# facebookresearch/brainmagick

Hardware: AMD Instinct MI355X
Metric: segments/s, 208-ch x 360-sample SimpleConv + ClipLoss training step (higher is better)
Workload: dtype f32 (fp32-accurate: operands split into 2 scaled f16 planes, 3 MFMA products, fp32 accumulate; same parity tolerances as exact fp32, see DESIGN.md §2); 1 GPU; cfg2: gwilliams2022-shaped MEG C=208 T=360, F=120 features, 27 subjects, clip_conv SimpleConv (8985590 params) + ClipLoss + Adam; batch_per_gpu=256, global_batch=256, negatives=local, parallelism=dp1, comm=none, rccl_world=1, candidate_gather=none, distinct_batches=8

## Files before the change

### brainmagick_amd/csrc/bm_common.h

```cpp
#pragma once
#include <hip/hip_runtime.h>
#include <stdint.h>
#include <stdio.h>
#include <math.h>

typedef float f32x16 __attribute__((ext_vector_type(16)));
typedef float f32x4 __attribute__((ext_vector_type(4)));

#define BM_OK 0
#define BM_ERR_ARG 1001
#define BM_ERR_WORKSPACE 1002
#define BM_ERR_UNSUPPORTED 1003

extern thread_local char bm_err_buf[512];
int bm_set_error(int code, const char* fmt, ...);
int bm_check_launch(const char* what);

#define BM_REQUIRE(cond, ...)                                   \
    do {                                                        \
        if (!(cond)) return bm_set_error(BM_ERR_ARG, __VA_ARGS__); \
    } while (0)

static inline int cdiv(long a, long b) { return (int)((a + b - 1) / b); }
static inline bool prefer_big(int n) { return (long)cdiv(n, 128) * 128 <= (long)cdiv(n, 64) * 64; }

struct BmFastDiv {
    unsigned mul, shift, d;
};
static inline BmFastDiv bm_fastdiv(unsigned d) {
    BmFastDiv f;
    f.d = d;
    unsigned l = 0;
    while ((1ull << l) < d) ++l;
    f.mul = (unsigned)((((1ull << l) - d) << 32) / d + 1);
    f.shift = l;
    return f;
}
__host__ __device__ __forceinline__ unsigned bm_div(unsigned n, const BmFastDiv& f) {
#if defined(__HIP_DEVICE_COMPILE__)
    const unsigned t = __umulhi(n, f.mul);
#else
    const unsigned t = (unsigned)(((unsigned long long)n * f.mul) >> 32);
#endif
    return f.shift == 0 ? n : (t + ((n - t) >> 1)) >> (f.shift - 1);
}
__host__ __device__ __forceinline__ int bm_floordiv(int a, int b) { return a >= 0 ? a / b : -((-a + b - 1) / b); }

#define BM_BKC 16
#define BM_WAVE 64

__device__ __forceinline__ int bm_xcd_remap(int id, int n) {
    const int q = n >> 3, r = n & 7;
    const int xcd = id & 7, slot = id >> 3;
    const int base = (xcd < r) ? xcd * (q + 1) : r * (q + 1) + (xcd - r) * q;
    return base + slot;
}

enum { BM_ACT_NONE = 0, BM_ACT_GELU = 1, BM_ACT_RELU = 2, BM_ACT_LEAKY = 3 };

__device__ __forceinline__ float bm_erff(float a) { return erff(a); }

__device__ __forceinline__ float bm_act(float z, int act, float leak) {
    if (act == BM_ACT_GELU) return 0.5f * z * (1.0f + bm_erff(z * 0.70710678118654752440f));
    if (act == BM_ACT_RELU) return !(z <= 0.f) ? z : 0.f;
    if (act == BM_ACT_LEAKY) return z > 0.f ? z : z * leak;
    return z;
}

__device__ __forceinline__ float bm_gelu_grad_fast(float z) {
    const float a = fabsf(z);
    const float t = __builtin_amdgcn_rcpf(fmaf(a, 0.24f, 1.0f));
    const float e = __builtin_amdgcn_exp2f(z * z * -0.72134752044448170368f);
    float q = -0.12508568359372038f;
    q = fmaf(q, t, 0.5545737304338939f);
    q = fmaf(q, t, -0.646070256151912f);
    q = fmaf(q, t, 0.6255898343952563f);
    q = fmaf(q, t, -0.15404857581855858f);
    q = fmaf(q, t, 0.15551350568092193f);
    q = fmaf(q, t, 0.08952744474497322f);
    const float eq = e * (q * t);
    const float base = z >= 0.f ? 1.0f - eq : eq;
    return fmaf(e, z * 0.39894228040143267794f, base);
}
#define BM_ACT_GELU_FASTGRAD 4

__device__ __forceinline__ float bm_act_grad(float z, int act, float leak) {
    if (act == BM_ACT_GELU_FASTGRAD) return bm_gelu_grad_fast(z);
    if (act == BM_ACT_GELU) {
        const float cdf = 0.5f * (1.0f + bm_erff(z * 0.70710678118654752440f));
        const float pdf = 0.39894228040143267794f * expf(-0.5f * z * z);
        return cdf + z * pdf;
    }
    if (act == BM_ACT_RELU) return !(z <= 0.f) ? 1.f : 0.f;
    if (act == BM_ACT_LEAKY) return z > 0.f ? 1.f : leak;
    return 1.f;
}

__device__ __forceinline__ float bm_wave_sum(float v) {
#pragma unroll
    for (int o = 32; o > 0; o >>= 1) v += __shfl_xor(v, o);
    return v;
}
__device__ __forceinline__ double bm_wave_sum_d(double v) {
#pragma unroll
    for (int o = 32; o > 0; o >>= 1) v += __shfl_xor(v, o);
    return v;
}
template <typename T>
__device__ __forceinline__ void bm_wave_to_lds(T v, T* sh) {
    if ((threadIdx.x & 63) == 0) sh[threadIdx.x >> 6] = v;
}
#define BM_AMAX_SHARDS 8
#define BM_AMAX_WS 16384
__device__ __forceinline__ float bm_wave_max(float v);
struct BmAmaxDst {
    float* ws;
};
__device__ __forceinline__ void bm_publish_amax_at(float m, const BmAmaxDst& dst, float* sh ,
                                                   unsigned wg ) {
    if (!dst.ws) return;
    bm_wave_to_lds(bm_wave_max(m), sh);
    __syncthreads();
    if (threadIdx.x == 0) {
        const int nw = (blockDim.x + 63) >> 6;
        float v = sh[0];
        for (int w = 1; w < nw; ++w) v = fmaxf(v, sh[w]);
        dst.ws[wg] = v;
    }
}
__device__ __forceinline__ void bm_publish_amax(float m, const BmAmaxDst& dst, float* sh) {
    bm_publish_amax_at(m, dst, sh, blockIdx.y * gridDim.x + blockIdx.x);
}
__device__ __forceinline__ void bm_publish_amax(float m, float* ws, float* sh) {
    bm_publish_amax(m, BmAmaxDst{ws}, sh);
}
__device__ __forceinline__ float bm_amax_load(const float* slot) {
    float m = slot[0];
#pragma unroll
    for (int i = 1; i < BM_AMAX_SHARDS; ++i) m = fmaxf(m, slot[i]);
    return m;
}
int bm_amax_finalize(const float* ws, int n, float* out, hipStream_t stream);
int bm_amax_finalize_rows(const float* ws, int C, int nsplit, float* out, float* rows_out, hipStream_t stream);
int bm_amax_finalize_rows_sums(const float* ws, int C, int nsplit, float* out, float* rows_out,
                               const double* sum_partial, float* sums_out, hipStream_t stream);
static inline BmAmaxDst bm_amax_dst(float* amax_out, float* amax_ws) {
    return BmAmaxDst{amax_out ? amax_ws : nullptr};
}
static inline int bm_amax_done(const BmAmaxDst& d, int nblocks, float* amax_out, hipStream_t stream) {
    return d.ws ? bm_amax_finalize(d.ws, nblocks, amax_out, stream) : BM_OK;
}

__device__ __forceinline__ float bm_wave_max(float v) {
#pragma unroll
    for (int o = 32; o > 0; o >>= 1) v = fmaxf(v, __shfl_xor(v, o));
    return v;
}
```

### brainmagick_amd/csrc/conv_h2_common.h

```cpp
#pragma once
#include <cstdlib>
#include <cstring>
#include "conv_common.h"
#include "mfma_split.h"

typedef _Float16 f16x8 __attribute__((ext_vector_type(8)));

#define HBN 192
#define HXWP 256
#define HXSLAB (2 * 2 * HXWP)
#define PACK_MAX_NK 3840

struct ConvH2Args {
    ConvNNArgs c;
    const float* x_amax;
    const float* wscale;
    BmAmaxDst y_amax;
};

template <int MW>
struct H2Simple {
    float* yb;
    const float* rb;
    int rowu, li, T;
    int row0, M;
    float bia[MW][16];
};

template <int MW, int NT, int MT, bool FULL>
__device__ __forceinline__ float h2_simple_col(const H2Simple<MW>& e, f32x16 (&acc)[MW][3], float amx) {
    if constexpr (MT < MW) {
        float rv[16];
        if (e.rb) {
#pragma unroll
            for (int r = 0; r < 16; ++r) {
                const int dr = MT * 32 + (r & 3) + 8 * (r >> 2);
                rv[r] = (FULL || e.row0 + dr < e.M) ? e.rb[(long)(e.rowu + dr) * e.T + e.li + NT * 32] : 0.f;
            }
        }
#pragma unroll
        for (int r = 0; r < 16; ++r) {
            const int dr = MT * 32 + (r & 3) + 8 * (r >> 2);
            float v = acc[MT][NT][r] + e.bia[MT][r];
            if (e.rb) v += rv[r];
            if (FULL || e.row0 + dr < e.M) {
                amx = fmaxf(amx, fabsf(v));
                e.yb[(long)(e.rowu + dr) * e.T + e.li + NT * 32] = v;
            }
        }
        return h2_simple_col<MW, NT, MT + 1, FULL>(e, acc, amx);
    }
    return amx;
}

template <int MW, bool FULL>
__device__ __forceinline__ float h2_simple_tile(const H2Simple<MW>& e, f32x16 (&acc)[MW][3], int col0, int T) {
    float amx = 0.f;
    if (col0 < T) amx = h2_simple_col<MW, 0, 0, FULL>(e, acc, amx);
    if (col0 + 32 < T) amx = h2_simple_col<MW, 1, 0, FULL>(e, acc, amx);
    if (col0 + 64 < T) amx = h2_simple_col<MW, 2, 0, FULL>(e, acc, amx);
    return amx;
}

struct H2Plain {
    float* yb;
    const float* rb;
    int rowu, li, T;
    int row0, M;
};

template <int MW, bool FULL>
__device__ __forceinline__ void h2_residual_add(const H2Plain& e, f32x16 (&acc)[MW][3], int col0, int T) {
    constexpr int NBLK = MW * 3, D = 3;
    float rv[D][16];
    const bool cok[3] = {col0 < T, col0 + 32 < T, col0 + 64 < T};
    bm_static_for<NBLK + D>([&](auto ic) __attribute__((always_inline)) {
        constexpr int i = decltype(ic)::value;
        if constexpr (i >= D) {
            constexpr int b = i - D, nt = b / MW, mt = b % MW;
            if (cok[nt]) {
#pragma unroll
                for (int r = 0; r < 16; ++r) acc[mt][nt][r] += rv[b % D][r];
            }
        }
        if constexpr (i < NBLK) {
            constexpr int nt = i / MW, mt = i % MW;
            if (cok[nt]) {
#pragma unroll
                for (int r = 0; r < 16; ++r) {
                    const int dr = mt * 32 + (r & 3) + 8 * (r >> 2);
                    rv[i % D][r] = (FULL || e.row0 + dr < e.M) ? e.rb[(long)(e.rowu + dr) * e.T + e.li + nt * 32] : 0.f;
                }
            }
        }
    });
}
template <int MW, int NT, int MT, bool FULL>
__device__ __forceinline__ float h2_plain_col(const H2Plain& e, f32x16 (&acc)[MW][3], float amx) {
    if constexpr (MT < MW) {
#pragma unroll
        for (int r = 0; r < 16; ++r) {
            const int dr = MT * 32 + (r & 3) + 8 * (r >> 2);
            const float v = acc[MT][NT][r];
            if (FULL || e.row0 + dr < e.M) {
                amx = fmaxf(amx, fabsf(v));
                e.yb[(long)(e.rowu + dr) * e.T + e.li + NT * 32] = v;
            }
        }
        return h2_plain_col<MW, NT, MT + 1, FULL>(e, acc, amx);
    }
    return amx;
}
template <int MW, bool FULL>
__device__ __forceinline__ float h2_plain_tile(const H2Plain& e, f32x16 (&acc)[MW][3], int col0, int T) {
    float amx = 0.f;
    if (col0 < T) amx = h2_plain_col<MW, 0, 0, FULL>(e, acc, amx);
    if (col0 + 32 < T) amx = h2_plain_col<MW, 1, 0, FULL>(e, acc, amx);
    if (col0 + 64 < T) amx = h2_plain_col<MW, 2, 0, FULL>(e, acc, amx);
    return amx;
}

template <int MW, int I>
__device__ __forceinline__ float h2_general_blocks(const ConvNNArgs& a, f32x16 (&acc)[MW][3], const float* ep, int b,
                                                   int m0, int rl_base, int col_base, float amx) {
    if constexpr (I < MW * 3) {
        constexpr int MT = I / 3, NT = I % 3;
        float v[16];
        float m = 0.f;
        conv_ep_store_block(a, acc[MT][NT], ep, 64 * MW, b, m0, rl_base + MT * 32, col_base + NT * 32, v, &m);
        return h2_general_blocks<MW, I + 1>(a, acc, ep, b, m0, rl_base, col_base, fmaxf(amx, m));
    }
    return amx;
}

template <int MW>
__device__ __forceinline__ void h2_tile_stats(const ConvNNArgs& a, f32x16 (&acc)[MW][3], const float* epl ,
                                              float* stats_tile , long row_stride ,
                                              int row0 , int col0, int lane) {
    const bool c0ok = col0 < a.T, c1ok = col0 + 32 < a.T, c2ok = col0 + 64 < a.T;
    const bool all_in = __builtin_amdgcn_readfirstlane(col0 - (lane & 31)) + 95 < a.T;
    const bool b4 = lane & 16, b3 = lane & 8, b2 = lane & 4, b1 = lane & 2;
    bm_static_for<MW>([&](auto mc) __attribute__((always_inline)) {
        constexpr int mt = decltype(mc)::value;
        float s1[16], s2[16];
        if (all_in) {
#pragma unroll
            for (int r = 0; r < 16; ++r) {
                const float bias = epl[mt * 32 + (r & 3) + 8 * (r >> 2)];
                const float v0 = acc[mt][0][r] + bias, v1 = acc[mt][1][r] + bias, v2 = acc[mt][2][r] + bias;
                s1[r] = (v0 + v1) + v2;
                s2[r] = fmaf(v0, v0, fmaf(v1, v1, v2 * v2));
            }
        } else {
#pragma unroll
            for (int r = 0; r < 16; ++r) {
                const float bias = epl[mt * 32 + (r & 3) + 8 * (r >> 2)];
                const float v0 = c0ok ? acc[mt][0][r] + bias : 0.f;
                const float v1 = c1ok ? acc[mt][1][r] + bias : 0.f;
                const float v2 = c2ok ? acc[mt][2][r] + bias : 0.f;
                s1[r] = (v0 + v1) + v2;
                s2[r] = fmaf(v0, v0, fmaf(v1, v1, v2 * v2));
            }
        }
#define H2_FOLD(N_, BIT_, MASK_)                                                                  \
        _Pragma("unroll") for (int i = 0; i < N_; ++i) {                                          \
            const float k1 = BIT_ ? s1[i + N_] : s1[i], g1 = BIT_ ? s1[i] : s1[i + N_];            \
            const float k2 = BIT_ ? s2[i + N_] : s2[i], g2 = BIT_ ? s2[i] : s2[i + N_];            \
            s1[i] = k1 + __shfl_xor(g1, MASK_);                                                   \
            s2[i] = k2 + __shfl_xor(g2, MASK_);                                                   \
        }
        H2_FOLD(8, b4, 16)
        H2_FOLD(4, b3, 8)
        H2_FOLD(2, b2, 4)
        H2_FOLD(1, b1, 2)
#undef H2_FOLD
        s1[0] += __shfl_xor(s1[0], 1);
        s2[0] += __shfl_xor(s2[0], 1);
        const int q = (b4 ? 8 : 0) + (b3 ? 4 : 0) + (b2 ? 2 : 0) + (b1 ? 1 : 0);
        const int row = row0 + mt * 32 + (q & 3) + 8 * (q >> 2);
        if (!(lane & 1) && row < a.M)
            *reinterpret_cast<float2*>(stats_tile + (long)row * row_stride) = float2{s1[0], s2[0]};
    });
}

template <int MW, bool RESK = false>
__device__ __forceinline__ void h2_tile_epilogue(const ConvH2Args& args, f32x16 (&acc)[MW][3], float* smem, int b, int g,
                                                 int m0, int n0, int ntile, float sx_inv, int tid, int lane, int wm,
                                                 int wn, int nl, int h, unsigned* trace_out = nullptr) {
    const ConvNNArgs& a = args.c;
    constexpr int NW = 3;
    constexpr int HBM = 64 * MW;
#ifdef HG_TRACE
    unsigned te[6];
#define H2_TE(I_) { __builtin_amdgcn_sched_barrier(0); te[I_] = (unsigned)__builtin_readcyclecounter(); __builtin_amdgcn_sched_barrier(0); }
#else
#define H2_TE(I_)
#endif
    H2_TE(0)
    float* ep = smem;
    conv_ep_stage_params(a, ep, HBM, m0, tid, 256, b);
    {
        const float* ws = args.wscale + (long)g * a.Mpad + m0;
        for (int i = tid; i < HBM; i += 256) ep[3 * HBM + i] = ws[i] * sx_inv;
    }
    __syncthreads();
    H2_TE(1)
    if constexpr (RESK) {
        const float* fl = ep + 3 * HBM + wm * (MW * 32) + 4 * h;
        const float* bl = ep + wm * (MW * 32) + 4 * h;
#pragma unroll
        for (int mt = 0; mt < MW; ++mt)
#pragma unroll
            for (int r = 0; r < 16; ++r) {
                const float f = fl[mt * 32 + (r & 3) + 8 * (r >> 2)];
                const float bb = bl[mt * 32 + (r & 3) + 8 * (r >> 2)];
#pragma unroll
                for (int nt = 0; nt < NW; ++nt) acc[mt][nt][r] = fmaf(acc[mt][nt][r], f, bb);
            }
        H2Plain e;
        e.yb = a.y_out + (long)b * a.y_bstride;
        e.rb = a.res + (long)b * a.res_bstride;
        e.rowu = m0 + wm * (MW * 32);
        e.li = 4 * h * a.T + n0 + wn * (NW * 32) + nl;
        e.T = a.T;
        e.row0 = e.rowu + 4 * h;
        e.M = a.M;
        const int col0 = n0 + wn * (NW * 32) + nl;
        float amx;
        if (m0 + HBM <= a.M) {
            h2_residual_add<MW, true>(e, acc, col0, a.T);
            amx = h2_plain_tile<MW, true>(e, acc, col0, a.T);
        } else {
            h2_residual_add<MW, false>(e, acc, col0, a.T);
            amx = h2_plain_tile<MW, false>(e, acc, col0, a.T);
        }
        bm_publish_amax(amx, args.y_amax, smem + 4 * HBM);
        return;
    }
    {
        const float* fl = ep + 3 * HBM + wm * (MW * 32) + 4 * h;
#pragma unroll
        for (int mt = 0; mt < MW; ++mt)
#pragma unroll
            for (int r = 0; r < 16; ++r) {
                const float f = fl[mt * 32 + (r & 3) + 8 * (r >> 2)];
#pragma unroll
                for (int nt = 0; nt < NW; ++nt) acc[mt][nt][r] *= f;
            }
    }
    H2_TE(2)
    if (a.stats)
        h2_tile_stats<MW>(a, acc, ep + wm * (MW * 32) + 4 * h,
                          a.stats + (long)((b * a.ntiles_n + ntile) * 2 + wn) * 2, (long)a.B * a.ntiles_n * 4,
                          m0 + wm * (MW * 32) + 4 * h, n0 + wn * (NW * 32) + nl, lane);
    const bool simple = ((a.y_pre != nullptr) != (a.y_out != nullptr)) && !a.ep_scale && a.act == BM_ACT_NONE;
    H2_TE(3)
    if (simple) {
        H2Simple<MW> e;
        e.yb = (a.y_pre ? a.y_pre : a.y_out) + (long)b * a.y_bstride;
        e.rb = (a.y_out && a.res) ? a.res + (long)b * a.res_bstride : nullptr;
        e.rowu = m0 + wm * (MW * 32);
        e.li = 4 * h * a.T + n0 + wn * (NW * 32) + nl;
        e.T = a.T;
        e.row0 = e.rowu + 4 * h;
        e.M = a.M;
        const float* epl = ep + wm * (MW * 32) + 4 * h;
#pragma unroll
        for (int mt = 0; mt < MW; ++mt)
#pragma unroll
            for (int r = 0; r < 16; ++r) e.bia[mt][r] = epl[mt * 32 + (r & 3) + 8 * (r >> 2)];
        const int col0 = n0 + wn * (NW * 32) + nl;
        const float amx = m0 + HBM <= a.M ? h2_simple_tile<MW, true>(e, acc, col0, a.T)
                                          : h2_simple_tile<MW, false>(e, acc, col0, a.T);
        H2_TE(4)
        if (a.y_out) bm_publish_amax(amx, args.y_amax, smem + 4 * HBM);
        H2_TE(5)
#ifdef HG_TRACE
        if (trace_out && blockIdx.x < 64 && lane == 0) {
            unsigned* o = trace_out + ((blockIdx.x * 4 + (threadIdx.x >> 6)) * 3) * 8;
            o[1] = te[1] - te[0]; o[2] = te[2] - te[1]; o[3] = te[3] - te[2]; o[8 + 1] = te[4] - te[3]; o[8 + 2] = te[5] - te[4];
        }
#endif
    } else {
        const float amx = h2_general_blocks<MW, 0>(a, acc, ep, b, m0, wm * (MW * 32) + 4 * h,
                                                   n0 + wn * (NW * 32) + nl, 0.f);
        bm_publish_amax(amx, args.y_amax, smem + 4 * HBM);
    }
}


#ifdef HG_TRACE
#define CH_T(I_) { __builtin_amdgcn_sched_barrier(0); tr[I_] = (unsigned)__builtin_readcyclecounter(); __builtin_amdgcn_sched_barrier(0); }
#else
#define CH_T(I_)
#endif

extern "C" int bm_conv_h2_mpad(int M);
extern "C" int bm_amax(const float* x, long n, float* out, float* ws, void* stream);
```

### brainmagick_amd/csrc/conv_nn_h2w.hip

```cpp
#include "conv_h2_common.h"

#ifdef HG_TRACE
__device__ unsigned ch_trace_buf[64 * 4 * 24];
extern "C" int bm_debug_trace_read_conv(unsigned* out) {
    return (int)hipMemcpyFromSymbol(out, HIP_SYMBOL(ch_trace_buf), sizeof(unsigned) * 64 * 4 * 24);
}
#endif

__device__ __forceinline__ void ch_split_hi(float x0, float x1, float s, unsigned& hi) {
    asm("v_fma_mixlo_f16 %0, %1, %3, 0\n\t"
        "v_fma_mixhi_f16 %0, %2, %3, 0" : "=&v"(hi) : "v"(x0), "v"(x1), "v"(s));
}
__device__ __forceinline__ void ch_split_lo(float x0, float x1, float s, unsigned hi, unsigned& lo) {
    asm("v_fma_mixlo_f16 %0, %2, %4, -%1 op_sel_hi:[0,0,1]\n\t"
        "v_fma_mixhi_f16 %0, %3, %4, -%1 op_sel:[0,0,1] op_sel_hi:[0,0,1]"
        : "=&v"(lo) : "v"(hi), "v"(x0), "v"(x1), "v"(s));
}

enum { H2R_NONE = 0, H2R_WLOAD, H2R_SPLIT, H2R_WRITE, H2R_BAR, H2R_BREAD };
struct H2RItem { int kind, arg; };
template <int KS, int J, int NB>
constexpr int h2r_nitems() {
    if (KS == 1) return 32 + 4 + 1 + NB;
    return J == 0 ? 16 + NB : J == 1 ? 16 + 4 + 1 + NB : NB;
}
template <int KS, int J, int NB>
constexpr H2RItem h2r_item(int i) {
    if (KS == 1) {
        if (i < 16) return (i & 3) < 2 ? H2RItem{H2R_SPLIT, (i >> 2) * 2 + (i & 1)} : H2RItem{H2R_WLOAD, (i >> 2) * 2 + (i & 1)};
        if (i < 18) return H2RItem{H2R_WRITE, i - 16};
        if (i < 34) { const int k = i - 18; return (k & 3) < 2 ? H2RItem{H2R_SPLIT, 8 + (k >> 2) * 2 + (k & 1)} : H2RItem{H2R_WLOAD, 8 + (k >> 2) * 2 + (k & 1)}; }
        if (i < 36) return H2RItem{H2R_WRITE, i - 34 + 2};
        if (i == 36) return H2RItem{H2R_BAR, 0};
        return H2RItem{H2R_BREAD, i - 37};
    }
    if (J == 0) return i < 16 ? H2RItem{H2R_WLOAD, i} : H2RItem{H2R_BREAD, i - 16};
    if (J == 1) {
        if (i < NB) return H2RItem{H2R_BREAD, i};
        i -= NB;
        if (i < 8) return H2RItem{H2R_SPLIT, i};
        if (i < 10) return H2RItem{H2R_WRITE, i - 8};
        if (i < 18) return H2RItem{H2R_SPLIT, i - 2};
        if (i < 20) return H2RItem{H2R_WRITE, i - 18 + 2};
        return H2RItem{H2R_BAR, 0};
    }
    return H2RItem{H2R_BREAD, i};
}

template <int KS, int MW, bool RESK = false>
__global__ __launch_bounds__(256, 1) void conv_nn_h2w_kernel(ConvH2Args args) {
    const ConvNNArgs& a = args.c;
#ifdef HG_TRACE
    const unsigned t_kernel0 = (unsigned)__builtin_readcyclecounter();
#endif
    constexpr int NW = 3;
    constexpr int HBM = 64 * MW;
    constexpr int TN = MW * NW, NS = 3 * TN;
    constexpr int NA = 2 * MW, NB = 2 * NW;
    constexpr int NF = NS - (NS + 3) / 4;
    static_assert(4 * (NA - 1) < NS, "the A loads of a stage need a slot each");
    extern __shared__ __attribute__((aligned(16))) float smem[];
    u32x4* Xs = reinterpret_cast<u32x4*>(smem);
    const int tid = threadIdx.x;
    const int lane = tid & 63;
    const int wave = __builtin_amdgcn_readfirstlane(tid >> 6);
    const int wm = wave >> 1, wn = wave & 1;
    const int nl = lane & 31;
    const int h = lane >> 5;

    int id = bm_xcd_remap(blockIdx.x, gridDim.x);
    const int mtile = id % a.ntiles_m;
    id /= a.ntiles_m;
    const int ntile = id % a.ntiles_n;
    const int b = id / a.ntiles_n;
    const int m0 = mtile * HBM;
    const int n0 = ntile * HBN;
    const int halo = (KS >> 1) * a.dil;
    const int XW = HBN + 2 * halo;

    const int g = a.widx ? a.widx[b] : 0;
    const int n16 = 2 * a.nchunk;
    float sx, sx_inv;
    bm_scale_from_amax(bm_amax_load(args.x_amax), sx, sx_inv);

    const long gslots = (long)a.nchunk * KS * 8 * a.Mpad;
    const __amdgpu_buffer_rsrc_t wr = bm_buffer_rsrc(reinterpret_cast<const u32x4*>(a.wp) + (long)g * gslots, (unsigned)(gslots * 16));
    const int wvoff = (h * a.Mpad + m0 + wm * (MW * 32) + nl) * 16;
    const int pstride = 4 * a.Mpad * 16;
    const __amdgpu_buffer_rsrc_t xr = bm_buffer_rsrc(a.x + (long)b * a.x_bstride, (unsigned)(a.Cin * a.T * 4));
    const int tcol = n0 - halo + tid;
    const int xoff0 = (tid < XW && tcol >= 0 && tcol < a.T) ? tcol * 4 : 0x40000000;
    const int crow = a.T * 4;

    f32x16 acc[MW][NW];
#pragma unroll
    for (int i = 0; i < MW; ++i)
#pragma unroll
        for (int k = 0; k < NW; ++k)
#pragma unroll
            for (int r = 0; r < 16; ++r) acc[i][k][r] = 0.f;

    float xreg[16];
    unsigned ph[8], pw[8];
    f16x8 af[2][2][MW], bf[2][2][NW];

#define H2R_LOAD_A(SET_, K_, SOFF_)                                                                       \
    af[SET_][1 - (K_) / MW][(K_) % MW] = __builtin_bit_cast(f16x8, __builtin_amdgcn_raw_buffer_load_b128(  \
        wr, wvoff + ((K_) % MW) * 512, (SOFF_) + (1 - (K_) / MW) * pstride, 0));
#define H2R_SOFF(C16_, J_) (((((C16_) >> 1) * KS + (J_)) * 8 + ((C16_) & 1) * 2) * a.Mpad * 16)
#define H2R_LOAD_X(R_, CB_) xreg[R_] = __builtin_bit_cast(float, __builtin_amdgcn_raw_buffer_load_b32(xr, (CB_) + (R_) * crow, 0, 0));
    const u32x4* xrd = Xs + h * HXWP + wn * (NW * 32) + nl;
    u32x4* xwr = Xs + tid;

    bm_static_for<16>([&](auto rc) __attribute__((always_inline)) { H2R_LOAD_X(decltype(rc)::value, xoff0) });
    bm_static_for<NA>([&](auto kc) __attribute__((always_inline)) { H2R_LOAD_A(0, decltype(kc)::value, 0) });
    bm_static_for<8>([&](auto uc) __attribute__((always_inline)) {
        constexpr int u = decltype(uc)::value;
        ch_split_hi(xreg[2 * u], xreg[2 * u + 1], sx, ph[u]);
        ch_split_lo(xreg[2 * u], xreg[2 * u + 1], sx, ph[u], pw[u]);
    });
    xwr[(0 * 2 + 0) * HXWP] = u32x4{ph[0], ph[1], ph[2], ph[3]};
    xwr[(1 * 2 + 0) * HXWP] = u32x4{pw[0], pw[1], pw[2], pw[3]};
    xwr[(0 * 2 + 1) * HXWP] = u32x4{ph[4], ph[5], ph[6], ph[7]};
    xwr[(1 * 2 + 1) * HXWP] = u32x4{pw[4], pw[5], pw[6], pw[7]};
    if (KS == 1) bm_static_for<16>([&](auto rc) __attribute__((always_inline)) { H2R_LOAD_X(decltype(rc)::value, 16 * crow + xoff0) });
    asm volatile("s_waitcnt lgkmcnt(0)\n\ts_barrier" ::: "memory");
    bm_static_for<NB>([&](auto ic) __attribute__((always_inline)) {
        constexpr int i = decltype(ic)::value;
        bf[0][i / NW][i % NW] = __builtin_bit_cast(f16x8, xrd[(i / NW) * 2 * HXWP + (i % NW) * 32]);
    });

#ifdef HG_TRACE
    unsigned tr[8], tacc[3][8];
    for (int i = 0; i < 3; ++i) for (int k = 0; k < 8; ++k) tacc[i][k] = 0;
    __builtin_amdgcn_sched_barrier(0);
    const unsigned t_loop0 = (unsigned)__builtin_readcyclecounter();
#endif
    auto stage = [&](int c16, auto jc, auto pc) __attribute__((always_inline)) {
        constexpr int j = decltype(jc)::value, par = decltype(pc)::value;
        CH_T(0)
        const bool last_chunk = c16 + 1 >= n16;
        const int nc16 = (j == KS - 1 && !last_chunk) ? c16 + 1 : c16;
        const int soff = (j == KS - 1) ? H2R_SOFF(nc16, last_chunk ? KS - 1 : 0) : H2R_SOFF(c16, j + 1);
        const u32x4* xnext = xrd + ((j == KS - 1 ? c16 + 1 : c16) & 1) * HXSLAB + (j == KS - 1 ? 0 : (j + 1) * a.dil);
        const int cb = (c16 + (KS == 1 ? 2 : 1)) * 16 * crow + xoff0;
        u32x4* xw = xwr + ((c16 + 1) & 1) * HXSLAB;
        bm_static_for<NS>([&](auto nc) __attribute__((always_inline)) {
            constexpr int n = decltype(nc)::value;
            constexpr int term = n / TN, w = n % TN, mt = w / NW, nt = w % NW;
            constexpr int pa = term == 0 ? 1 : 0, pb = term == 1 ? 1 : 0;
            acc[mt][nt] = __builtin_amdgcn_mfma_f32_32x32x16_f16(af[par][pa][mt], bf[par][pb][nt], acc[mt][nt], 0, 0, 0);
            if constexpr (n % 4 == 0) {
                if constexpr (n / 4 < NA) H2R_LOAD_A(par ^ 1, n / 4, soff)
            } else {
                constexpr int f = (n / 4) * 3 + n % 4 - 1;
                constexpr int L = h2r_nitems<KS, j, NB>();
                constexpr int i0 = (f * L + NF - 1) / NF, i1 = ((f + 1) * L + NF - 1) / NF;
                bm_static_for<i1 - i0>([&](auto ic) __attribute__((always_inline)) {
                    constexpr H2RItem it = h2r_item<KS, j, NB>(i0 + decltype(ic)::value);
                    if constexpr (it.kind == H2R_WLOAD) {
                        H2R_LOAD_X(it.arg, cb)
                    } else if constexpr (it.kind == H2R_SPLIT) {
                        constexpr int u = it.arg / 2;
                        if constexpr (it.arg % 2 == 0) ch_split_hi(xreg[2 * u], xreg[2 * u + 1], sx, ph[u]);
                        else ch_split_lo(xreg[2 * u], xreg[2 * u + 1], sx, ph[u], pw[u]);
                    } else if constexpr (it.kind == H2R_WRITE) {
                        constexpr int kg = it.arg / 2, plane = it.arg % 2;
                        if constexpr (plane == 0) xw[(0 * 2 + kg) * HXWP] = u32x4{ph[4 * kg], ph[4 * kg + 1], ph[4 * kg + 2], ph[4 * kg + 3]};
                        else xw[(1 * 2 + kg) * HXWP] = u32x4{pw[4 * kg], pw[4 * kg + 1], pw[4 * kg + 2], pw[4 * kg + 3]};
                    } else if constexpr (it.kind == H2R_BAR) {
                        asm volatile("s_waitcnt lgkmcnt(0)\n\ts_barrier" ::: "memory");
                    } else if constexpr (it.kind == H2R_BREAD) {
                        constexpr int p = it.arg / NW, q = it.arg % NW;
                        bf[par ^ 1][p][q] = __builtin_bit_cast(f16x8, xnext[p * 2 * HXWP + q * 32]);
                    }
                });
            }
            __builtin_amdgcn_sched_barrier(0);
        });
        CH_T(4)
#ifdef HG_TRACE
        tacc[j][0] += tr[4] - tr[0]; tacc[j][7] += 1;
#endif
    };
    auto chunk = [&](int c16, auto cpc) __attribute__((always_inline)) {
        constexpr int cp = decltype(cpc)::value;
        bm_static_for<KS>([&](auto jc) __attribute__((always_inline)) {
            constexpr int j = decltype(jc)::value;
            stage(c16, jc, std::integral_constant<int, (cp + j) & 1>{});
        });
    };
    for (int c16 = 0; c16 < n16; c16 += 2) {
        chunk(c16, std::integral_constant<int, 0>{});
        chunk(c16 + 1, std::integral_constant<int, KS & 1>{});
    }
#ifdef HG_TRACE
    __builtin_amdgcn_sched_barrier(0);
    const unsigned t_loop1 = (unsigned)__builtin_readcyclecounter();
    if (blockIdx.x < 64 && lane == 0)
        for (int i = 0; i < 3; ++i) for (int k = 0; k < 8; ++k) ch_trace_buf[((blockIdx.x * 4 + wave) * 3 + i) * 8 + k] = tacc[i][k];
#endif
    asm volatile("s_waitcnt vmcnt(0) lgkmcnt(0)\n\ts_barrier" ::: "memory");
#undef H2R_LOAD_A
#undef H2R_SOFF
#undef H2R_LOAD_X

#ifdef HG_TRACE
    h2_tile_epilogue<MW, RESK>(args, acc, smem, b, g, m0, n0, ntile, sx_inv, tid, lane, wm, wn, nl, h, ch_trace_buf);
#else
    h2_tile_epilogue<MW, RESK>(args, acc, smem, b, g, m0, n0, ntile, sx_inv, tid, lane, wm, wn, nl, h);
#endif
#ifdef HG_TRACE
    asm volatile("s_waitcnt vmcnt(0)" ::: "memory");
    if (blockIdx.x < 64 && lane == 0) {
        unsigned* o = ch_trace_buf + ((blockIdx.x * 4 + wave) * 3) * 8;
        o[5] = t_loop0 - t_kernel0;
        o[6] = (unsigned)__builtin_readcyclecounter() - t_loop1;
        o[8 + 5] = t_loop1 - t_loop0;
    }
#endif
}

extern "C" int bm_conv_h2_mw_for(int M) {
    int best = 5;
    long best_pad = -1;
    const int cand[3] = {5, 4, 2};
    for (int i = 0; i < 3; ++i) {
        const long bm = 64L * cand[i];
        const long pad = (long)cdiv(M, bm) * bm;
        if (best_pad < 0 || pad < best_pad) { best_pad = pad; best = cand[i]; }
    }
    return best;
}
extern "C" int bm_conv_h2_mpad(int M) {
    const int bm = 64 * bm_conv_h2_mw_for(M);
    return cdiv(M, bm) * bm;
}

extern "C" int bm_conv_h2_covers(int Cin, int M, int T, int KS, int dil) {
    if (KS != 1 && KS != 3) return 0;
    if ((KS >> 1) * dil > 16 || T <= 128) return 0;
    if ((long)Cin * T * 4 >= 0x40000000L) return 0;
    if ((long)Cin * KS > PACK_MAX_NK) return 0;
    return (long)bm_conv_h2_mpad(M) * 2 <= (long)M * 3 || M >= 96;
}

extern "C" int bm_conv_h2_stats_tiles(int B, int T) { return B * cdiv(T, HBN) * 2; }

template <int KS, int MW>
static int launch_conv_nn_h2w(ConvH2Args args, float* y_amax_out, hipStream_t stream) {
    constexpr int HBM = 64 * MW;
    const size_t lds_ep = (size_t)(4 * HBM + 4) * sizeof(float);
    const size_t lds = (size_t)(2 * HXSLAB) * 16 > lds_ep ? (size_t)(2 * HXSLAB) * 16 : lds_ep;
    const ConvNNArgs& c = args.c;
    const bool resk = KS == 3 && c.res && c.y_out && !c.y_pre && !c.ep_scale && !c.stats && c.act == BM_ACT_NONE;
    args.c.ntiles_n = cdiv(args.c.T, HBN);
    args.c.ntiles_m = args.c.Mpad / HBM;
    const long nblocks = (long)args.c.B * args.c.ntiles_n * args.c.ntiles_m;
    if (nblocks <= 0) return BM_OK;
    const bool publish = y_amax_out && args.y_amax.ws && nblocks <= BM_AMAX_WS;
    float* ws = args.y_amax.ws;
    if (!publish) args.y_amax = BmAmaxDst{nullptr};
    if (resk)
        hipLaunchKernelGGL((conv_nn_h2w_kernel<KS, MW, KS == 3>), dim3((unsigned)nblocks), dim3(256), lds, stream, args);
    else
        hipLaunchKernelGGL((conv_nn_h2w_kernel<KS, MW, false>), dim3((unsigned)nblocks), dim3(256), lds, stream, args);
    if (int rc = bm_check_launch("conv_nn_h2w")) return rc;
    if (publish) return bm_amax_done(args.y_amax, (int)nblocks, y_amax_out, stream);
    if (y_amax_out && ws)
        return bm_amax(args.c.y_out, (long)args.c.B * args.c.M * args.c.T, y_amax_out, ws, stream);
    return BM_OK;
}

extern "C" int bm_conv1d_nn_h2(const float* x, long x_bstride, const float* x_amax, const void* wpacked,
                               const int* widx, const float* bias, long bias_gstride, const float* ep_scale, const float* ep_shift,
                               const float* res, long res_bstride, float* y_pre, float* y_out, long y_bstride,
                               float* stats, int B, int Cin, int M, int T, int KS, int dil, int act, float leak,
                               int G, float* y_amax_out, float* amax_ws, void* stream) {
    BM_REQUIRE(x_amax, "conv1d_nn_h2: null x_amax");
    BM_REQUIRE(G >= 1, "conv1d_nn_h2: bad dims");
    BM_REQUIRE(!stats || (y_pre && !y_out && !ep_scale && act == BM_ACT_NONE && !res),
               "conv1d_nn_h2: per-tile statistics come with y_pre alone (the training-mode BatchNorm layers)");
    ConvH2Args args;
    ConvNNArgs& a = args.c;
    if (int e = conv_nn_fill_args(a, "conv1d_nn_h2", x, x_bstride, (const float*)wpacked, widx, bias, bias_gstride, ep_scale,
                                  ep_shift, res, res_bstride, y_pre, y_out, y_bstride, stats, B, Cin, M, T, KS, dil, act,
                                  leak))
        return e;
    BM_REQUIRE(bm_conv_h2_covers(Cin, M, T, KS, dil), "conv1d_nn_h2: shape not covered (Cin=%d M=%d T=%d KS=%d dil=%d)",
               Cin, M, T, KS, dil);
    const int mw = bm_conv_h2_mw_for(M);
    a.Mpad = bm_conv_h2_mpad(M);
    a.nchunk = cdiv(Cin, 32);
    const long f16_elems = (long)G * a.nchunk * KS * 2 * 4 * a.Mpad * 8;
    args.x_amax = x_amax;
    BM_REQUIRE(!y_amax_out || amax_ws, "conv1d_nn_h2: y_amax_out needs the amax workspace");
    if (!y_out) y_amax_out = nullptr;
    args.y_amax = bm_amax_dst(y_amax_out, amax_ws);
    args.wscale = reinterpret_cast<const float*>(reinterpret_cast<const char*>(wpacked) + f16_elems * 2);
    hipStream_t s = (hipStream_t)stream;
#define H2_DISPATCH(MW_)                                                                 \
    return KS == 1 ? launch_conv_nn_h2w<1, MW_>(args, y_amax_out, s) : launch_conv_nn_h2w<3, MW_>(args, y_amax_out, s);
    switch (mw) {
        case 5: H2_DISPATCH(5)
        case 4: H2_DISPATCH(4)
        default: H2_DISPATCH(2)
    }
#undef H2_DISPATCH
}
```

### brainmagick_amd/csrc/core.hip

```cpp
#include "bm_block.h"
#include <stdarg.h>
#include <stdlib.h>

thread_local char bm_err_buf[512] = {0};

int bm_set_error(int code, const char* fmt, ...) {
    va_list ap;
    va_start(ap, fmt);
    vsnprintf(bm_err_buf, sizeof(bm_err_buf), fmt, ap);
    va_end(ap);
    return code;
}

int bm_check_launch(const char* what) {
    hipError_t e = hipGetLastError();
    if (e != hipSuccess) return bm_set_error((int)e, "%s: launch failed: %s", what, hipGetErrorString(e));
    return BM_OK;
}

extern "C" const char* bm_last_error(void) { return bm_err_buf; }
extern "C" int bm_version(void) { return 116; }

extern "C" int bm_device_count(void) {
    int n = 0;
    hipError_t e = hipGetDeviceCount(&n);
    if (e != hipSuccess) { bm_set_error((int)e, "hipGetDeviceCount: %s", hipGetErrorString(e)); return -1; }
    return n;
}

#define FIN_THREADS 1024
#define FIN_WAVES (FIN_THREADS / 64)
__global__ __launch_bounds__(FIN_THREADS) void amax_finalize_kernel(const float* __restrict__ ws, int n,
                                                                    float* __restrict__ out) {
    __shared__ float sh[FIN_WAVES];
    bm_amax_fold<FIN_WAVES>(ws, n, out, sh);
}

int bm_amax_finalize(const float* ws, int n, float* out, hipStream_t stream) {
    if (!out) return BM_OK;
    hipLaunchKernelGGL(amax_finalize_kernel, dim3(1), dim3(FIN_THREADS), 0, stream, ws, n, out);
    return bm_check_launch("amax_finalize");
}

__global__ __launch_bounds__(FIN_THREADS) void amax_finalize_rows_kernel(const float* __restrict__ ws, int C, int nsplit,
                                                                         float* __restrict__ out,
                                                                         float* __restrict__ rows_out,
                                                                         const double* __restrict__ sum_partial,
                                                                         float* __restrict__ sums_out) {
    __shared__ float sh[FIN_WAVES];
    if (sum_partial)
        for (int c = threadIdx.x; c < C; c += FIN_THREADS) {
            double t = 0;
            for (int s = 0; s < nsplit; ++s) t += sum_partial[(long)c * nsplit + s];
            sums_out[c] = (float)t;
        }
    bm_amax_fold_rows<FIN_WAVES>(ws, C, nsplit, 1, C, out, rows_out, sh);
}

int bm_amax_finalize_rows(const float* ws, int C, int nsplit, float* out, float* rows_out, hipStream_t stream) {
    if (!out) return BM_OK;
    hipLaunchKernelGGL(amax_finalize_rows_kernel, dim3(1), dim3(FIN_THREADS), 0, stream, ws, C, nsplit, out, rows_out,
                       (const double*)nullptr, (float*)nullptr);
    return bm_check_launch("amax_finalize_rows");
}

int bm_amax_finalize_rows_sums(const float* ws, int C, int nsplit, float* out, float* rows_out,
                               const double* sum_partial, float* sums_out, hipStream_t stream) {
    hipLaunchKernelGGL(amax_finalize_rows_kernel, dim3(1), dim3(FIN_THREADS), 0, stream, ws, C, nsplit, out, rows_out,
                       sum_partial, sums_out);
    return bm_check_launch("amax_finalize_rows");
}

extern "C" int bm_amax_ws_elems(void) { return BM_AMAX_WS; }
```

### brainmagick_amd/functional.py

```python

import torch

from . import hip_ops as H



ACT_CODES = {"none": H.ACT_NONE, "gelu": H.ACT_GELU, "relu": H.ACT_RELU, "leaky": H.ACT_LEAKY}


def _c(t: torch.Tensor) -> torch.Tensor:
    return t if t.is_contiguous() else t.contiguous()


_arange_cache = {}


def _arange_i32(n: int, device, repeat: int = 1) -> torch.Tensor:
    key = (n, repeat, device.type, device.index)
    t = _arange_cache.get(key)
    if t is None:
        if len(_arange_cache) > 64:
            _arange_cache.clear()
        t = torch.arange(n, dtype=torch.int32, device=device)
        if repeat != 1:
            t = t.repeat(repeat)
        if device.type == "cuda":
            torch.cuda.current_stream(device).synchronize()
        _arange_cache[key] = t
    return t


def _conv_weight_grads(dy, x, weight, KS, dil, transposed_weight):
    dst = H.grad_destination(weight)
    B, M, T = dy.shape
    Cin = x.shape[1]
    if transposed_weight:
        out = dst if dst is not None else torch.empty(weight.shape, device=dy.device, dtype=torch.float32)
        H.gemm_nt(x, dy, B, Cin, M, T, 1, 1, out=out.view(1, Cin, M, 1))
        return out.view(weight.shape) if dst is not None else out
    if dst is not None:
        H.gemm_nt(dy, x, B, M, Cin, T, KS, dil, out=dst.view(1, M, Cin, KS))
        return dst.view(weight.shape)
    return H.gemm_nt(dy, x, B, M, Cin, T, KS, dil).view(weight.shape)


def _layer_forward(x, weight, geom, res=None, **kw):
    dil, transposed, stride, pad = geom
    if pad is not None:
        assert res is None, "the strided family has no fused residual"
        KS = weight.shape[2]
        M = weight.shape[1] if transposed else weight.shape[0]
        Tout = H.conv_out_len(x.shape[2], KS, stride, dil, pad, transposed)
        wp = H.pack_strided_rows_second(weight) if transposed else H.pack_strided_rows_first(weight)
        return H.conv_strided(x, wp, M, Tout, KS, stride, dil, pad, transposed, **kw)
    assert stride == 1
    if transposed:
        Cin, M, KS = weight.shape
        assert KS == 1, "ConvTranspose1d is only supported with kernel 1 (simpleconv.py:189)"
        wp = H.pack_weights(weight, 1, M, Cin, 1, 0, 1, M, 0, shape=(x.shape[2], dil))
    else:
        M, Cin, KS = weight.shape
        wp = H.pack_conv_fwd(weight, (x.shape[2], dil))
    if kw.get("want_stats") and getattr(wp, "_bm_mode", "") != "f16x2":
        pre, out, _ = H.conv_nn(x, wp, M, KS, dil, res=res, **dict(kw, want_stats=False))
        return pre, out, H.channel_stats(pre)
    return H.conv_nn(x, wp, M, KS, dil, res=res, **kw)


def _layer_backward(ctx, dy, x, weight, geom, res=None, publish_amax=True):
    dil, transposed, stride, pad = geom
    KS = weight.shape[2]
    Cin, T = x.shape[1], x.shape[2]
    dw = None
    if ctx.needs_input_grad[1]:
        if pad is None:
            dw = _conv_weight_grads(dy, x, weight, KS, dil, transposed)
        else:
            a, xl = (x, dy) if transposed else (dy, x)
            dw = H.conv_strided_wgrad(a, xl, KS, stride, dil, pad, out=H.grad_destination(weight)).view(weight.shape)
    dx = None
    if ctx.needs_input_grad[0]:
        if pad is not None:
            wp = H.pack_strided_rows_first(weight) if transposed else H.pack_strided_rows_second(weight)
            _, dx, _ = H.conv_strided(dy, wp, Cin, T, KS, stride, dil, pad, not transposed)
        else:
            if transposed:
                M = weight.shape[1]
                wp = H.pack_weights(weight, 1, Cin, M, 1, 0, M, 1, 0, shape=(T, dil))
            else:
                wp = H.pack_conv_dgrad(weight, (T, dil))
            _, dx, _ = H.conv_nn(dy, wp, Cin, KS, dil, res=res, publish_amax=publish_amax)
    return dx, dw


class Conv1dFn(torch.autograd.Function):

    @staticmethod
    def forward(ctx, x, weight, bias, dil: int, act: int, leak: float, transposed_weight: bool, stride: int = 1,
                pad=None):
        x, weight = _c(x), _c(weight)
        geom = (dil, transposed_weight, stride, pad)
        need_pre = act != H.ACT_NONE and any(ctx.needs_input_grad[:3])
        if need_pre and pad is None:
            pre, _, _ = _layer_forward(x, weight, geom, bias=bias, want_pre=True, want_out=False)
            out = H.affine_act_res(pre, None, None, None, act, leak)
        else:
            pre, out, _ = _layer_forward(x, weight, geom, bias=bias, act=act, leak=leak, want_pre=need_pre)
        ctx.save_for_backward(x, weight, pre)
        ctx.cfg = (geom, act, leak, bias is not None)
        return out

    @staticmethod
    def backward(ctx, dout):
        x, weight, pre = ctx.saved_tensors
        geom, act, leak, has_bias = ctx.cfg
        dout = _c(dout)
        dbias = None
        if act != H.ACT_NONE:
            dy, _, _, dbias = H.act_bn_bwd(dout, pre, None, None, None, None, False, act, leak,
                                           want_dbias=has_bias)
        else:
            dy = dout
            if has_bias:
                dbias = H.channel_sum(dy)
        dx, dw = _layer_backward(ctx, dy, x, weight, geom)
        return (dx, dw, dbias) + (None,) * 6


class ConvBNActFn(torch.autograd.Function):

    @staticmethod
    def forward(ctx, x, weight, bias, gamma, beta, running_mean, running_var, num_batches,
                training: bool, dil: int, act: int, leak: float, residual: bool, momentum: float,
                eps: float, stride: int = 1, pad=None, transposed: bool = False):
        x, weight = _c(x), _c(weight)
        geom = (dil, transposed, stride, pad)
        res = x if residual else None
        needs_grad = any(ctx.needs_input_grad[:5])
        if training:
            pre, _, stats = _layer_forward(x, weight, geom, bias=bias, want_pre=True, want_out=False, want_stats=True)
            mean, invstd, scale, shift = H.bn_finalize(stats, pre.shape[0] * pre.shape[2], gamma, beta, running_mean,
                                                       running_var, num_batches, momentum, eps)
            out = H.affine_act_res(pre, scale, shift, res, act, leak)
        else:
            mean, invstd, scale, shift = H.bn_eval_affine(gamma, beta, running_mean, running_var, eps)
            pre, out, _ = _layer_forward(x, weight, geom, res=res, bias=bias, scale=scale, shift=shift, act=act,
                                         leak=leak, want_pre=needs_grad)
        ctx.save_for_backward(x, weight, pre, scale, shift, mean, invstd)
        ctx.cfg = (geom, training, act, leak, residual, bias is not None)
        return out

    @staticmethod
    def backward(ctx, dout):
        x, weight, pre, scale, shift, mean, invstd = ctx.saved_tensors
        geom, training, act, leak, residual, has_bias = ctx.cfg
        dout = _c(dout)
        dy, dgamma, dbeta, dbias = H.act_bn_bwd(dout, pre, scale, shift, mean, invstd, training, act,
                                                leak, want_affine_grads=True, want_dbias=has_bias)
        dx, dw = _layer_backward(ctx, dy, x, weight, geom, res=dout if residual else None, publish_amax=False)
        return (dx, dw, dbias, dgamma, dbeta) + (None,) * 13


class GLUConvFn(torch.autograd.Function):

    @staticmethod
    def forward(ctx, x, weight, bias):
        x, weight = _c(x), _c(weight)
        M, Cin, KS = weight.shape
        u, _, _ = H.conv_nn(x, H.pack_conv_fwd(weight, (x.shape[2], 1)), M, KS, 1, bias=bias, want_pre=True,
                            want_out=False)
        out = H.glu_fwd(u)
        ctx.save_for_backward(x, weight, u)
        ctx.has_bias = bias is not None
        return out

    @staticmethod
    def backward(ctx, dout):
        x, weight, u = ctx.saved_tensors
        M, Cin, KS = weight.shape
        du, dbias = H.glu_bwd(_c(dout), u, want_dbias=ctx.has_bias)
        dw = _conv_weight_grads(du, x, weight, KS, 1, False) if ctx.needs_input_grad[1] else None  
        dx = None
        if ctx.needs_input_grad[0]:
            _, dx, _ = H.conv_nn(du, H.pack_conv_dgrad(weight, (du.shape[2], 1)), Cin, KS, 1, publish_amax=False)
        return dx, dw, dbias


class SubjectLayersFn(torch.autograd.Function):

    @staticmethod
    def forward(ctx, x, weights, subjects):
        x, weights = _c(x), _c(weights)
        S, C, D = weights.shape
        widx = H.index_i32(_c(subjects.to(torch.int64)), S)
        wp = H.pack_weights(weights, S, D, C, 1, C * D, 1, D, 0, shape=(x.shape[2], 1))
        _, out, _ = H.conv_nn(x, wp, D, 1, 1, widx=widx)
        ctx.save_for_backward(x, weights, subjects, widx)
        return out

    @staticmethod
    def backward(ctx, dout):
        x, weights, subjects, widx = ctx.saved_tensors
        S, C, D = weights.shape
        dout = _c(dout)
        B, _, T = x.shape
        dx = None
        if ctx.needs_input_grad[0]:
            wpt = H.pack_weights(weights, S, C, D, 1, C * D, D, 1, 0, shape=(T, 1))
            _, dx, _ = H.conv_nn(dout, wpt, C, 1, 1, widx=widx)
        dw = None
        if ctx.needs_input_grad[1]:
            order, seg = H.group_by_index(_c(subjects.to(torch.int64)), S)
            dw = torch.empty_like(weights)
            H.gemm_nt(dout, x, B, D, C, T, 1, 1, order=order, seg=seg, G=S, out=dw,
                      out_strides=(C * D, 1, D, 0))
        return dx, dw, None


class ChannelMergerFn(torch.autograd.Function):

    @staticmethod
    def forward(ctx, meg, heads, positions_u, layout_index, ban_center, ban_radius: float):
        meg, heads, positions_u = _c(meg), _c(heads), _c(positions_u)
        U, C, _ = positions_u.shape
        O, D = heads.shape[-2:]
        per_layout_heads = heads.dim() == 3
        assert not per_layout_heads or heads.shape[0] == U
        emb = H.fourier_emb(positions_u, D)
        seg = _arange_i32(U + 1, meg.device)
        scores = H.gemm_nt(heads, emb, U, O, C, D, a_strides=(O * D if per_layout_heads else 0, D),
                           x_strides=(C * D, D), seg=seg, G=U).view(U, O, C)
        weights = H.masked_softmax(scores, positions_u, ban_center, ban_radius)
        widx = H.index_i32(_c(layout_index.to(torch.int64)), U)
        wp = H.pack_weights(weights, U, O, C, 1, O * C, C, 1, 0, shape=(meg.shape[2], 1))
        _, out, _ = H.conv_nn(meg, wp, O, 1, 1, widx=widx)
        ctx.save_for_backward(meg, emb, weights, layout_index, widx)
        ctx.dims = (U, C, O, D)
        ctx.per_layout_heads = per_layout_heads
        return out

    @staticmethod
    def backward(ctx, dout):
        meg, emb, weights, layout_index, widx = ctx.saved_tensors
        U, C, O, D = ctx.dims
        dout = _c(dout)
        B, _, T = meg.shape
        dheads = None
        if ctx.needs_input_grad[1]:
            order, seg = H.group_by_index(_c(layout_index.to(torch.int64)), U)
            dweights = H.gemm_nt(dout, meg, B, O, C, T, 1, 1, order=order, seg=seg, G=U).view(U, O, C)
            dscores = H.softmax_bwd(weights, dweights)
            wp = H.pack_weights(dscores, U, O, C, 1, O * C, C, 1, 0, shape=(D, 1))
            uidx = _arange_i32(U, meg.device)
            _, per_layout, _ = H.conv_nn(emb, wp, O, 1, 1, widx=uidx)
            if ctx.per_layout_heads:
                dheads = per_layout
            else:
                dheads = H.sum_over_batch(per_layout) if U > 1 else per_layout[0]
        dmeg = None
        if ctx.needs_input_grad[0]:
            wpt = H.pack_weights(weights, U, C, O, 1, O * C, 1, C, 0, shape=(T, 1))
            _, dmeg, _ = H.conv_nn(dout, wpt, C, 1, 1, widx=widx)
        return dmeg, dheads, None, None, None, None


class FusedFrontEndFn(torch.autograd.Function):

    @staticmethod
    def forward(ctx, meg, heads, w1, b1, ws, positions_u, layout_index, subjects, ban_center, ban_radius: float):
        meg, heads, w1, ws, positions_u = _c(meg), _c(heads), _c(w1), _c(ws), _c(positions_u)
        U, C, _ = positions_u.shape
        O, Dp = heads.shape
        L = w1.shape[0]
        S, _, D = ws.shape
        B, _, T = meg.shape
        dev = meg.device
        emb = H.fourier_emb(positions_u, Dp)
        seg_u = _arange_i32(U + 1, dev)
        scores = H.gemm_nt(heads, emb, U, O, C, Dp, a_strides=(0, Dp), x_strides=(C * Dp, Dp), seg=seg_u,
                           G=U).view(U, O, C)
        wm = H.masked_softmax(scores, positions_u, ban_center, ban_radius)
        _, p, _ = H.conv_nn(wm, H.pack_conv_fwd(w1), L, 1, 1)
        bcol = (b1 if b1 is not None else torch.zeros(L, device=dev)).view(1, L, 1).expand(U, L, 1)
        xp = torch.cat([p, bcol], dim=2).repeat_interleave(S, dim=0).contiguous()
        widx_p = _arange_i32(S, dev, repeat=U)
        _, wc, _ = H.conv_nn(xp, H.pack_weights(ws, S, D, L, 1, L * D, 1, D, 0), D, 1, 1, widx=widx_p)
        bias_c = wc[:, :, C].contiguous()
        pair = H.index_i32(_c(layout_index.to(torch.int64)), U) * S + H.index_i32(_c(subjects.to(torch.int64)), S)
        wpc = H.pack_weights(wc, U * S, D, C, 1, D * (C + 1), C + 1, 1, 0, shape=(T, 1))
        _, out, _ = H.conv_nn(meg, wpc, D, 1, 1, widx=pair, bias=bias_c, bias_gstride=D)
        ctx.save_for_backward(meg, emb, wm, xp, ws, w1, pair, widx_p, wc)
        ctx.dims = (U, C, O, Dp, L, S, D)
        ctx.has_b1 = b1 is not None
        return out

    @staticmethod
    def backward(ctx, dout):
        meg, emb, wm, xp, ws, w1, pair, widx_p, wc = ctx.saved_tensors
        U, C, O, Dp, L, S, D = ctx.dims
        dout = _c(dout)
        B, _, T = meg.shape
        dev = meg.device
        P = U * S
        order, seg = H.group_by_index(pair.to(torch.int64), P)
        gaug = torch.empty(P, D, C + 1, device=dev, dtype=torch.float32)
        H.gemm_nt(dout, meg, B, D, C, T, 1, 1, order=order, seg=seg, G=P, out=gaug,
                  out_strides=(D * (C + 1), C + 1, 1, 0))
        gaug[:, :, C] = H.segment_sum_cols(H.time_sums_t(dout), order, seg).t()
        seg_p = _arange_i32(P + 1, dev)
        dws = dw1 = db1 = dheads = None
        if ctx.needs_input_grad[4]:
            t1 = H.gemm_nt(xp, gaug, P, L, D, C + 1, seg=seg_p, G=P)
            dws = (H.sum_over_batch(t1.view(U, S * L * D)) if U > 1 else t1).view(S, L, D)
        _, a, _ = H.conv_nn(gaug, H.pack_weights(ws, S, L, D, 1, L * D, D, 1, 0), L, 1, 1, widx=widx_p)
        a_u = torch.stack([H.sum_over_batch(a[u * S:(u + 1) * S]) for u in range(U)])
        if ctx.has_b1 and ctx.needs_input_grad[3]:
            db1 = H.sum_over_batch(a_u[:, :, C].contiguous()) if U > 1 else a_u[0, :, C].contiguous()
        if ctx.needs_input_grad[2]:
            dw1 = H.gemm_nt(a_u, wm, U, L, O, C, 1, 1, a_strides=(L * (C + 1), C + 1),
                            x_strides=(O * C, C)).view(L, O, 1)
        if ctx.needs_input_grad[1]:
            _, dwm, _ = H.conv_nn(a_u, H.pack_conv_dgrad(w1), O, 1, 1)
            dscores = H.softmax_bwd(wm, dwm[:, :, :C].contiguous())
            wp = H.pack_weights(dscores, U, O, C, 1, O * C, C, 1, 0, shape=(Dp, 1))
            uidx = _arange_i32(U, dev)
            _, per_layout, _ = H.conv_nn(emb, wp, O, 1, 1, widx=uidx)
            dheads = H.sum_over_batch(per_layout) if U > 1 else per_layout[0]
        dmeg = None
        if ctx.needs_input_grad[0]:
            wpt = H.pack_weights(wc, P, C, D, 1, D * (C + 1), 1, C + 1, 0, shape=(T, 1))
            _, dmeg, _ = H.conv_nn(dout, wpt, C, 1, 1, widx=pair)
        return dmeg, dheads, dw1, db1, dws, None, None, None, None, None


_CLIP_BLOCK_BYTES = 0x3f000000


def _candidate_blocks(Bc: int, K: int):
    if Bc * K * 4 < _CLIP_BLOCK_BYTES:
        return [(0, Bc)]
    rows = max(1, _CLIP_BLOCK_BYTES // (K * 4))
    if rows >= 128:
        rows -= rows % 128
    return [(r0, min(rows, Bc - r0)) for r0 in range(0, Bc, rows)]


def _clip_raw_scores(estimate, candidate, B, Bc, K):
    blocks = _candidate_blocks(Bc, K)
    if len(blocks) == 1:
        return H.gemm_nt_partials(estimate, candidate, 1, B, Bc, K, (0, K), (0, K))
    raw = torch.empty(1, B, Bc, device=estimate.device, dtype=torch.float32)
    cand2 = candidate.view(Bc, K)
    for r0, rows in blocks:
        blk = H.share_amax(candidate, cand2[r0:r0 + rows])
        H.gemm_nt(estimate, blk, 1, B, rows, K, 1, 1, a_strides=(0, K), x_strides=(0, K),
                  out=raw.view(-1)[r0:], out_strides=(0, Bc, 1, 0))
    return raw


class ClipLossFn(torch.autograd.Function):

    @staticmethod
    def forward(ctx, estimate, candidate, target_offset: int = 0, col_valid=None, symmetric: bool = False,
                normalize: bool = True):
        estimate, candidate = _c(estimate), _c(candidate)
        B, Bc = estimate.shape[0], candidate.shape[0]
        K = estimate.numel() // B
        assert candidate.numel() // Bc == K
        inv = H.clip_inv_norms(candidate) if normalize else torch.ones(Bc, device=candidate.device, dtype=torch.float32)
        ctx.normalize = normalize
        part = _clip_raw_scores(estimate, candidate, B, Bc, K)
        scores, _, dscaled, loss = H.clip_ce(part, inv, want_grad=True, want_loss=True,
                                             target_offset=target_offset, col_valid=col_valid)
        if symmetric:
            H.clip_ce_cols(scores, inv, dscaled, loss, target_offset=target_offset)
        if ctx.needs_input_grad[1]:
            ctx.save_for_backward(candidate, dscaled, estimate, scores, inv)
        else:
            ctx.save_for_backward(candidate, dscaled)
        ctx.shape = estimate.shape
        ctx.cand_shape = candidate.shape
        ctx.mark_non_differentiable(scores)
        return loss, scores

    @staticmethod
    def backward(ctx, dloss, _dscores):
        candidate, dscaled = ctx.saved_tensors[:2]
        B, Bc = dscaled.shape
        K = candidate.numel() // Bc
        alpha = _c(dloss).view(1)
        blocks = _candidate_blocks(Bc, K)
        cand2 = candidate.view(Bc, K)
        dest = None
        if ctx.needs_input_grad[0]:
            for r0, rows in blocks:
                wp = H.pack_weights(dscaled.view(-1)[r0:], 1, B, rows, 1, 0, Bc, 1, 0, alpha=alpha, shape=(K, 1))
                blk = H.share_amax(candidate, cand2[r0:r0 + rows].view(1, rows, K))
                _, dest, _ = H.conv_nn(blk, wp, B, 1, 1, res=dest, out=dest)
            dest = H.share_amax(dest, dest.view(ctx.shape))
        dcand = None
        if ctx.needs_input_grad[1]:
            estimate, scores, inv = ctx.saved_tensors[2:]
            dcand = torch.empty(Bc, K, device=candidate.device, dtype=torch.float32)
            for r0, rows in blocks:
                wpt = H.pack_weights(dscaled.view(-1)[r0:], 1, rows, B, 1, 0, 1, Bc, 0, alpha=alpha, shape=(K, 1))
                H.conv_nn(estimate.view(1, B, K), wpt, rows, 1, 1,
                          out=dcand[r0:r0 + rows] if len(blocks) > 1 else dcand)
            if ctx.normalize:
                coef = H.clip_cand_coef(dscaled, scores, inv, alpha)
                H.row_axpy_sub(dcand, cand2, coef)
            dcand = dcand.view(ctx.cand_shape)
        return dest, dcand, None, None, None, None


def clip_scores(estimate, candidate, want_probs=False):
    estimate, candidate = _c(estimate), _c(candidate)
    B, Bc = estimate.shape[0], candidate.shape[0]
    K = estimate.numel() // B
    inv = H.clip_inv_norms(candidate)
    part = _clip_raw_scores(estimate, candidate, B, Bc, K)
    scores, probs, _, _ = H.clip_ce(part, inv, want_probs=want_probs)
    return probs if want_probs else scores


def clip_forward_timed(estimate, candidate, inv, timer):
    B, Bc = estimate.shape[0], candidate.shape[0]
    K = estimate.numel() // B
    H.set_kernel_timer(timer)
    try:
        part = _clip_raw_scores(estimate, candidate, B, Bc, K)
        return H.clip_ce(part, inv, want_grad=True, want_loss=True)
    finally:
        H.set_kernel_timer(None)


class MaskedRegressionFn(torch.autograd.Function):

    @staticmethod
    def forward(ctx, estimate, output, mask, kind: str, flag=None):
        estimate, output = _c(estimate), _c(output)
        mask = None if mask is None else _c(mask)
        loss, count = H.regress_loss_fwd(estimate, output, mask, kind, flag)
        ctx.kind = kind
        ctx.save_for_backward(estimate, output, mask, count)
        ctx.mark_non_differentiable(count)
        return loss, count

    @staticmethod
    def backward(ctx, dloss, _dcount):
        estimate, output, mask, count = ctx.saved_tensors
        if not (ctx.needs_input_grad[0] or ctx.needs_input_grad[1]):
            return None, None, None, None, None
        dest, dout = H.regress_loss_bwd(estimate, output, mask, ctx.kind, _c(dloss), count,
                                        want_dout=ctx.needs_input_grad[1])
        return (dest if ctx.needs_input_grad[0] else None), dout, None, None, None


class FeatureDecodingFn(torch.autograd.Function):

    @staticmethod
    def forward(ctx, estimate, output, mask, table, weights=None, flag=None):
        estimate, output = _c(estimate), _c(output)
        mask = None if mask is None else _c(mask)
# ... 120 lines not shown
```

### brainmagick_amd/hip_ops.py

```python
import ctypes
import math
import typing as tp

import numpy as np
import torch

from ._lib import lib, check, BmHipError

ACT_NONE, ACT_GELU, ACT_RELU, ACT_LEAKY = 0, 1, 2, 3
BKC = 16

import os as _os
DEFAULT_COMPUTE_DTYPE = "f16x2"
COMPUTE_DTYPES = ("f32", "f32x3", "f16x2")
_compute_dtype = _os.environ.get("BM_COMPUTE_DTYPE", DEFAULT_COMPUTE_DTYPE)
if _compute_dtype not in COMPUTE_DTYPES:
    raise ValueError(f"BM_COMPUTE_DTYPE must be one of {COMPUTE_DTYPES}, got {_compute_dtype!r}")


def set_compute_dtype(name: str):
    global _compute_dtype
    if name not in COMPUTE_DTYPES:
        raise ValueError(f"compute dtype must be one of {COMPUTE_DTYPES}, got {name!r}")
    _compute_dtype = name


def get_compute_dtype() -> str:
    return _compute_dtype


class KernelTimer:

    def __init__(self):
        self.records: tp.List[tp.Tuple[str, float, torch.cuda.Event, torch.cuda.Event]] = []

    def launch(self, name: str, flops: float, fn):
        start = torch.cuda.Event(enable_timing=True)
        end = torch.cuda.Event(enable_timing=True)
        start.record()
        out = fn()
        end.record()
        self.records.append((name, flops, start, end))
        return out

    def summary(self) -> tp.Dict[str, tp.Dict[str, float]]:
        samples: tp.Dict[str, tp.List[float]] = {}
        flops_sum: tp.Dict[str, float] = {}
        for name, flops, start, end in self.records:
            samples.setdefault(name, []).append(start.elapsed_time(end))
            flops_sum[name] = flops_sum.get(name, 0.0) + flops
        out = {}
        for name, v in samples.items():
            med = sorted(v)[len(v) // 2]
            kept = [t for t in v if t <= 20.0 * med]
            out[name] = dict(launches=len(v), avg_ms=sum(kept) / len(kept), median_ms=med, max_ms=max(v),
                             outliers=len(v) - len(kept), flops_per_launch=flops_sum[name] / len(v))
        return out


_timer: tp.Optional[KernelTimer] = None
_MODE_SUFFIX = {"f32": "", "f32x3": "_x3", "f16x2": "_h2w"}


def set_kernel_timer(timer: tp.Optional[KernelTimer]):
    global _timer
    _timer = timer


def _timed(label, flops: float, launch):
    if _timer is None:
        return launch()
    return _timer.launch(label() if callable(label) else label, flops, launch)


def _p(t: tp.Optional[torch.Tensor]):
    return None if t is None else ctypes.c_void_p(t.data_ptr())


def _stream():
    return ctypes.c_void_p(torch.cuda.current_stream().cuda_stream)


def _req(t: torch.Tensor, name: str, dtype=torch.float32, contiguous: bool = True):
    if not isinstance(t, torch.Tensor) or not t.is_cuda:
        raise BmHipError(f"{name}: expected a GPU tensor; the brainmagick_amd hot path has no CPU "
                         "fallback (got %s)" % (t.device if isinstance(t, torch.Tensor) else type(t)))
    if t.dtype != dtype:
        raise BmHipError(f"{name}: expected dtype {dtype}, got {t.dtype}")
    if contiguous and not t.is_contiguous():
        raise BmHipError(f"{name}: expected a contiguous tensor")
    return t


def _opt(t, name, dtype=torch.float32):
    return None if t is None else _req(t, name, dtype)


_WS_KINDS = {
    "amax": ("bm_amax_ws_elems", torch.float32, False),
    "regress": ("bm_regress_workspace_bytes", torch.uint8, True),
    "encode": ("bm_meg_init_workspace_bytes", torch.uint8, True),
    "lowpass": ("bm_lowpass_workspace_bytes", torch.uint8, True),
}
_stream_workspaces: tp.Dict[tp.Any, torch.Tensor] = {}


def _stream_ws(kind: str, device) -> torch.Tensor:
    key = (kind, device, torch.cuda.current_stream(device).cuda_stream)
    ws = _stream_workspaces.get(key)
    if ws is None:
        size, dtype, zeroed = _WS_KINDS[kind]
        alloc = torch.zeros if zeroed else torch.empty
        ws = _stream_workspaces[key] = alloc(getattr(lib(), size)(), device=device, dtype=dtype)
    return ws


def conv_mpad(M: int) -> int:
    return lib().bm_conv_mpad(M)


def _note(t: torch.Tensor, attr: str, value, *checked):
    try:
        setattr(t, attr, (t._version, t.data_ptr(), value) + checked)
        t._bm_epoch = _weights_epoch
    except Exception:
        pass


def _noted(t: torch.Tensor, attr: str, need_checked: bool = False):
    note = getattr(t, attr, None)
    if note is not None and note[0] == t._version and note[1] == t.data_ptr() and (not need_checked or note[3]) and \
            (not (t.requires_grad and t.is_leaf) or getattr(t, "_bm_epoch", None) == _weights_epoch):
        return note[2]
    return None


AMAX_SHARDS = 8
amax_scans = 0


def amax(x: torch.Tensor, nonfinite_flag: tp.Optional[torch.Tensor] = None) -> torch.Tensor:
    cached = _noted(x, "_bm_amax", nonfinite_flag is not None)
    if cached is not None:
        return cached
    _req(x, "amax.x")
    global amax_scans
    amax_scans += 1
    out = torch.empty(AMAX_SHARDS, device=x.device, dtype=torch.float32)
    check(lib().bm_amax_checked(_p(x), x.numel(), _p(out), _p(_stream_ws("amax", x.device)),
                                _p(_opt(nonfinite_flag, "nonfinite_flag", torch.int32)), _stream()), "bm_amax")
    _note(x, "_bm_amax", out, nonfinite_flag is not None)
    return out


_amax_pool: tp.Dict[torch.device, tp.List[tp.Any]] = {}


def _amax_slot(t: torch.Tensor) -> tp.Optional[torch.Tensor]:
    if _compute_dtype != "f16x2" or t.numel() == 0:
        return None
    pool = _amax_pool.get(t.device)
    if pool is None or pool[1] >= pool[0].numel():
        pool = _amax_pool[t.device] = [torch.zeros(4096 * AMAX_SHARDS, device=t.device, dtype=torch.float32), 0]
    slot = pool[0][pool[1]:pool[1] + AMAX_SHARDS]
    pool[1] += AMAX_SHARDS
    _note(t, "_bm_amax", slot, False)
    return slot


def _row_amax_out(t: torch.Tensor, slot) -> tp.Optional[torch.Tensor]:
    if slot is None:
        return None
    rows = torch.empty(t.shape[1], device=t.device, dtype=torch.float32)
    _note(t, "_bm_row_amax", rows)
    return rows


def row_amax_of(t: torch.Tensor) -> tp.Optional[torch.Tensor]:
    return _noted(t, "_bm_row_amax")


def _slot_args(slot):
    return (_p(slot), _p(_stream_ws("amax", slot.device)) if slot is not None else None)


def _touched(t: torch.Tensor) -> torch.Tensor:
    for attr in ("_bm_amax", "_bm_row_amax", "_bm_inv_norms"):
        if getattr(t, attr, None) is not None:
            try:
                delattr(t, attr)
            except AttributeError:
                pass
    return t


def share_amax(src: torch.Tensor, view: torch.Tensor) -> torch.Tensor:
    if _compute_dtype != "f16x2":
        return view
    _note(view, "_bm_amax", amax(src), False)
    return view


_weights_epoch = 0
pack_launches = 0


def weights_changed():
    global _weights_epoch
    _weights_epoch += 1


class _PackPlan:
    MAX_JOBS = 512
    KEEP = 3

    def __init__(self, device):
        self.device = device
        self.entries: tp.Dict[tuple, dict] = {}
        self.table: tp.Optional[torch.Tensor] = None
        self.total_blocks = 0

    def get(self, src: torch.Tensor, geom: tuple) -> torch.Tensor:
        key = (src.data_ptr(),) + geom
        e = self.entries.get(key)
        if e is None:
            if len(self.entries) >= self.MAX_JOBS:
                self.entries.clear()
            G, M, Cin, KS = geom[:4]
            dst = torch.empty(lib().bm_packed_weight_bytes_h2(G, M, Cin, KS), device=src.device, dtype=torch.uint8)
            dst._bm_mode = "f16x2"
            dst._bm_groups = G
            e = self.entries[key] = dict(src=src, ptr=src.data_ptr(), geom=geom, dst=dst, stamp=None)
            self.table = None
        e["used"] = _weights_epoch
        if e["stamp"] != (_weights_epoch, src._version):
            self.refresh()
        return e["dst"]

    def refresh(self):
        global pack_launches
        stale = [k for k, e in self.entries.items()
                 if e["used"] < _weights_epoch - self.KEEP or e["src"].data_ptr() != e["ptr"]]
        for k in stale:
            del self.entries[k]
        if stale:
            self.table = None
        ents = list(self.entries.values())
        if not ents:
            return
        if self.table is None:
            nb = lib().bm_pack_h2_job_bytes()
            host = ctypes.create_string_buffer(nb * len(ents))
            block0 = 0
            for i, e in enumerate(ents):
                n = lib().bm_pack_h2_job_fill(ctypes.c_void_p(ctypes.addressof(host) + i * nb), _p(e["src"]),
                                              _p(e["dst"]), *e["geom"], None, block0)
                if n < 0:
                    raise BmHipError("bm_pack_h2_job_fill: bad arguments %r" % (e["geom"],))
                block0 += n
            self.table = torch.frombuffer(bytearray(host.raw), dtype=torch.uint8).to(self.device)
            self.total_blocks = block0
        max_nk = max(e["geom"][2] * e["geom"][3] for e in ents)
        check(lib().bm_pack_weights_h2_batch(_p(self.table), len(ents), self.total_blocks, max_nk, _stream()),
              "bm_pack_weights_h2_batch")
        pack_launches += 1
        for e in ents:
            e["stamp"] = (_weights_epoch, e["src"]._version)


_pack_plans: tp.Dict[tp.Tuple[str, int], _PackPlan] = {}


def _pack_plan(device) -> _PackPlan:
    key = (device.type, device.index if device.index is not None else torch.cuda.current_device())
    if key not in _pack_plans:
        _pack_plans[key] = _PackPlan(torch.device(*key))
    return _pack_plans[key]


def pack_weights(src: torch.Tensor, G: int, M: int, Cin: int, KS: int, sg: int, sm: int, sc: int,
                 sj: int, flip: bool = False, alpha: tp.Optional[torch.Tensor] = None,
                 shape: tp.Optional[tp.Tuple[int, int]] = None) -> torch.Tensor:
    _req(src, "pack_weights.src")
    mode = _compute_dtype
    if mode == "f16x2":
        if shape is not None and lib().bm_conv_h2_covers(Cin, M, shape[0], KS, shape[1]):
            if alpha is None and src.requires_grad and src.is_leaf:
                return _pack_plan(src.device).get(src, (G, M, Cin, KS, sg, sm, sc, sj, int(flip)))
            nbytes = lib().bm_packed_weight_bytes_h2(G, M, Cin, KS)
            dst = torch.empty(nbytes, device=src.device, dtype=torch.uint8)
            check(lib().bm_pack_weights_h2(_p(src), _p(dst), G, M, Cin, KS, sg, sm, sc, sj, int(flip),
                                           _p(_opt(alpha, "alpha")), _stream()), "bm_pack_weights_h2")
            global pack_launches
            pack_launches += 1
            dst._bm_mode = "f16x2"
            dst._bm_groups = G
            return dst
        mode = "f32x3"
    if mode == "f32x3":
        n = lib().bm_packed_weight_elems_x3(G, M, Cin, KS)
        dst = torch.empty(n, device=src.device, dtype=torch.bfloat16)
        check(lib().bm_pack_weights_x3(_p(src), _p(dst), G, M, Cin, KS, sg, sm, sc, sj, int(flip),
                                       _p(_opt(alpha, "alpha")), _stream()), "bm_pack_weights_x3")
        dst._bm_mode = mode
        return dst
    return pack_weights_f32(src, M, Cin, KS, sm, sc, sj, G, sg, flip, alpha)


def pack_weights_f32(src: torch.Tensor, M: int, Cin: int, KS: int, sm: int, sc: int, sj: int, G: int = 1, sg: int = 0,
                     flip: bool = False, alpha: tp.Optional[torch.Tensor] = None) -> torch.Tensor:
    _req(src, "pack_weights_f32.src")
    dst = torch.empty(lib().bm_packed_weight_elems(G, M, Cin, KS), device=src.device, dtype=torch.float32)
    check(lib().bm_pack_weights(_p(src), _p(dst), G, M, Cin, KS, sg, sm, sc, sj, int(flip), _p(_opt(alpha, "alpha")),
                                _stream()), "bm_pack_weights")
    return dst


def pack_conv_fwd(weight: torch.Tensor, shape=None) -> torch.Tensor:
    M, Cin, KS = weight.shape
    return pack_weights(weight, 1, M, Cin, KS, 0, Cin * KS, KS, 1, shape=shape)


def pack_conv_dgrad(weight: torch.Tensor, shape=None) -> torch.Tensor:
    M, Cin, KS = weight.shape
    return pack_weights(weight, 1, Cin, M, KS, 0, KS, Cin * KS, 1, flip=True, shape=shape)


def _conv_outputs(x: torch.Tensor, M: int, T: int, want_pre: bool, want_out: bool, stats_shape=None):
    def new(shape, want=True):
        return torch.empty(shape, device=x.device, dtype=torch.float32) if want and shape is not None else None
    return new((x.shape[0], M, T), want_pre), new((x.shape[0], M, T), want_out), new(stats_shape)


def conv_nn(x: torch.Tensor, wpacked: torch.Tensor, M: int, KS: int = 1, dil: int = 1,
            widx: tp.Optional[torch.Tensor] = None, bias=None, scale=None, shift=None, res=None,
            act: int = ACT_NONE, leak: float = 0., want_pre: bool = False, want_out: bool = True,
            want_stats: bool = False, out: tp.Optional[torch.Tensor] = None, bias_gstride: int = 0,
            publish_amax: bool = True):
    _req(x, "conv_nn.x")
    mode = getattr(wpacked, "_bm_mode", "f32")
    _req(wpacked, "conv_nn.w", {"f32": torch.float32, "f16x2": torch.uint8}.get(mode, torch.bfloat16))
    B, Cin, T = x.shape
    channel_major = want_stats and mode == "f16x2"
    stats_shape = None if not want_stats else (M, lib().bm_conv_h2_stats_tiles(B, T), 2) if channel_major else \
        (lib().bm_conv_stats_tiles(B, T), M, 2)
    y_pre, y_out, stats = _conv_outputs(x, M, T, want_pre, want_out and out is None, stats_shape)
    if channel_major:
        stats._bm_channel_major = True
    if out is not None:
        _req(out, "conv_nn.out")
        assert want_out and out.numel() == B * M * T, (out.shape, (B, M, T))
        y_out = _touched(out)
    if res is not None:
        _req(res, "conv_nn.res")
        assert res.shape == (B, M, T), (res.shape, (B, M, T))
    common = (_p(_opt(widx, "widx", torch.int32)), _p(_opt(bias, "bias")), bias_gstride, _p(_opt(scale, "scale")),
              _p(_opt(shift, "shift")), _p(res), M * T, _p(y_pre), _p(y_out), M * T, _p(stats), B, Cin, M, T,
              KS, dil, act, leak)
    if mode == "f16x2":
        x_amax = amax(x)
        y_slot = _amax_slot(y_out) if (y_out is not None and publish_amax) else None

        def launch():
            check(lib().bm_conv1d_nn_h2(_p(x), Cin * T, _p(x_amax), _p(wpacked), *common, wpacked._bm_groups,
                                        *_slot_args(y_slot), _stream()), "bm_conv1d_nn_h2")
    else:
        fn = {"f32": lib().bm_conv1d_nn, "f32x3": lib().bm_conv1d_nn_x3}[mode]

        def launch():
            check(fn(_p(x), Cin * T, _p(wpacked), *common, _stream()), f"bm_conv1d_nn[{mode}]")

    def label():
        if mode == "f16x2":
            tile = f"{KS},{lib().bm_conv_h2_mw_for(M)}"
        else:
            tile = (lib().bm_conv_mt_for if mode == "f32" else lib().bm_conv_x3_mt_for)(M)
        return f"conv_nn{_MODE_SUFFIX[mode]}_kernel<{tile}>"
    _timed(label, 2.0 * B * T * M * Cin * KS, launch)
    return y_pre, y_out, stats


def conv_out_len(T: int, KS: int, stride: int, dil: int, pad: int, transposed: bool) -> int:
    Tout = lib().bm_conv1d_out_len(T, KS, stride, dil, pad, int(transposed))
    if Tout < 1:
        if transposed:
            raise RuntimeError(f"ConvTranspose1d: input of {T} samples (kernel {KS}, stride {stride}, dilation {dil}, "
                               f"padding {pad}) gives an output of {Tout} samples. Output size is too small")
        raise RuntimeError(f"Calculated padded input size per channel: ({T + 2 * pad}). Kernel size: "
                           f"({dil * (KS - 1) + 1}). Kernel size can't be greater than actual input size")
    return Tout


def pack_strided_rows_first(weight: torch.Tensor) -> torch.Tensor:
    R, C, KS = weight.shape
    return pack_weights_f32(weight, R, C, KS, C * KS, KS, 1)


def pack_strided_rows_second(weight: torch.Tensor) -> torch.Tensor:
    C, R, KS = weight.shape
    return pack_weights_f32(weight, R, C, KS, KS, R * KS, 1)


def conv_strided(x: torch.Tensor, wpacked: torch.Tensor, M: int, Tout: int, KS: int, stride: int, dil: int, pad: int,
                 transposed: bool, bias=None, scale=None, shift=None, act: int = ACT_NONE, leak: float = 0.,
                 want_pre: bool = False, want_out: bool = True, want_stats: bool = False):
    _req(x, "conv_strided.x")
    _req(wpacked, "conv_strided.w")
    B, Cin, T = x.shape
    if Tout < 1:
        raise RuntimeError(f"conv_strided: output length {Tout} < 1")
    y_pre, y_out, stats = _conv_outputs(
        x, M, Tout, want_pre, want_out,
        (lib().bm_conv_strided_stats_tiles(B, Tout, stride, int(transposed)), M, 2) if want_stats else None)
    fn = lib().bm_conv1d_transposed if transposed else lib().bm_conv1d_strided
    name = "conv_transposed_kernel" if transposed else "conv_strided_kernel"

    def launch():
        check(fn(_p(x), Cin * T, _p(wpacked), _p(_opt(bias, "bias")), _p(_opt(scale, "scale")), _p(_opt(shift, "shift")),
                 _p(y_pre), _p(y_out), M * Tout, _p(stats), B, Cin, M, T, Tout, KS, stride, dil, pad, act, leak,
                 _stream()), "bm_conv1d_transposed" if transposed else "bm_conv1d_strided")
    taps = KS if not transposed else -(-KS // stride)
    _timed(f"{name}<K={KS},s={stride}>", 2.0 * B * (Tout if not transposed else T * stride) * M * Cin * taps, launch)
    return y_pre, y_out, stats


def conv_strided_wgrad(a: torch.Tensor, xl: torch.Tensor, KS: int, stride: int, dil: int, pad: int,
                       out: tp.Optional[torch.Tensor] = None, nsplit: tp.Optional[int] = None) -> torch.Tensor:
    _req(a, "conv_strided_wgrad.a")
    _req(xl, "conv_strided_wgrad.xl")
    S, R, U = a.shape
    S2, Q, L = xl.shape
    assert S == S2, (a.shape, xl.shape)
    if out is None:
        out = torch.empty(R, Q, KS, device=a.device, dtype=torch.float32)
    else:
        _req(out, "conv_strided_wgrad.out")
        assert out.numel() == R * Q * KS
        _touched(out)
    if nsplit is None:
        nsplit = lib().bm_conv1d_strided_wgrad_suggest_splits(R, Q, KS, S, U)
    part = out if nsplit == 1 else torch.empty(nsplit * R * Q * KS, device=a.device, dtype=torch.float32)

    def launch():
        check(lib().bm_conv1d_strided_wgrad(_p(a), R * U, _p(xl), Q * L, _p(part), S, R, Q, U, L, KS, stride, dil, pad,
                                            nsplit, _stream()), "bm_conv1d_strided_wgrad")
    _timed(f"conv_strided_wgrad_kernel<K={KS},s={stride}>", 2.0 * S * U * R * Q * KS, launch)
    if part is not out:
        check(lib().bm_reduce_splits(_p(part), _p(out), 1, nsplit, R, Q, KS, R * Q * KS, Q * KS, KS, 1, _stream()),
              "bm_reduce_splits")
    return out


_index_err: tp.Dict[torch.device, torch.Tensor] = {}
_CHECK_INDICES_NOW = _os.environ.get("BM_CHECK_INDICES", "0") == "1"


def index_error_flag(device) -> torch.Tensor:
    device = torch.device(device)
    if device.index is None:
        device = torch.device("cuda", torch.cuda.current_device())
    flag = _index_err.get(device)
    if flag is None:
        flag = torch.zeros(3, device=device, dtype=torch.int32)
        _index_err[device] = flag
    return flag


def raise_if_index_error(device=None):
    flags = list(_index_err.values()) if device is None else [index_error_flag(device)]
    for flag in flags:
        if int(flag[0].item()) != 0:
            flag[0:1].zero_()
            raise IndexError("subject / layout index out of range for the weight table "
                             "(bm/models/common.py:57 would raise in `weights.gather`)")


def index_i32(idx: torch.Tensor, G: int) -> torch.Tensor:
    _req(idx, "index_i32.idx", torch.int64)
    out = torch.empty(idx.numel(), device=idx.device, dtype=torch.int32)
    check(lib().bm_index_to_i32(_p(idx), idx.numel(), G, _p(out), _p(index_error_flag(idx.device)),
                                _stream()), "bm_index_to_i32")
    if _CHECK_INDICES_NOW:
        raise_if_index_error(idx.device)
    return out


def group_by_index(idx: torch.Tensor, G: int):
    _req(idx, "group_by_index.idx", torch.int64)
    B = idx.numel()
    order = torch.empty(B, device=idx.device, dtype=torch.int32)
    seg = torch.empty(G + 1, device=idx.device, dtype=torch.int32)
    check(lib().bm_group_by_index(_p(idx), B, G, _p(order), _p(seg), _p(index_error_flag(idx.device)),
                                  _stream()), "bm_group_by_index")
    return order, seg


_NT_SUFFIX = {"f32": "", "f32x3": "_x3"}


def _nt_plan(M, Cn, KS, S, T, G, dil, grouped, a_strides, x_strides, nsplit=None, partials=False):
    L = lib()
    family, swapped = _compute_dtype, False
    if family == "f16x2":
        family = "f32x3"
        if partials:
            if L.bm_gemm_nt_h2_covers(M, Cn, 1, S, T, 1, 1, 0):
                dense = S == 1 and tuple(a_strides) == (0, T) and tuple(x_strides) == (0, T)
                family = "scores" if dense and L.bm_clip_scores_h2_covers(M, Cn, T) else "h2"
        elif a_strides[1] == T and x_strides[1] == T and \
                (S == 1 or (a_strides[0] == M * T and x_strides[0] == Cn * T)):
            covered = bool(L.bm_gemm_nt_h2_covers(M, Cn, KS, S, T, G, dil, int(grouped)))
            swapped = not covered and KS == 1 and bool(L.bm_gemm_nt_h2_covers(Cn, M, KS, S, T, G, dil, int(grouped)))
            if swapped:
                M, Cn = Cn, M
            if covered or swapped:
                family = "h2_grouped" if grouped else "h2_rows"
    if nsplit is None:
        if family == "scores":
            nsplit = L.bm_clip_scores_h2_suggest_splits(M, Cn, T)
        elif partials:
            nsplit = L.bm_gemm_nt_h2_suggest_splits(M, Cn, 1, S, T) if family == "h2" else \
                L.bm_clip_suggest_splits(M, Cn, S, T)
        elif family in _NT_SUFFIX:
            nsplit = L.bm_gemm_nt_suggest_splits(M, Cn, KS, S, T, G)
        else:
            nsplit = L.bm_gemm_nt_h2_suggest_splits_grouped(M, Cn, KS, S, T, G)
    return family, swapped, nsplit


def _nt_launch(family, label, a, x, part, S, G, M, Cn, T, KS, dil, a_strides, x_strides, order, seg, nsplit):
    L = lib()
    if family in _NT_SUFFIX:
        fn = L.bm_gemm_nt if family == "f32" else L.bm_gemm_nt_x3

        def launch():
            check(fn(_p(a), a_strides[0], a_strides[1], _p(x), x_strides[0], x_strides[1],
                     _p(_opt(order, "order", torch.int32)), _p(_opt(seg, "seg", torch.int32)), _p(part), S,
                     G, M, Cn, T, KS, dil, nsplit, _stream()), "bm_gemm_nt")
    else:
        a_amax, x_amax = amax(a), amax(x)
        a_rows = row_amax_of(a) if family == "h2_rows" else None
        if a_rows is not None and a_rows.numel() != M:
            a_rows = None

        def launch():
            if family == "scores":
                check(L.bm_clip_scores_h2(_p(a), _p(a_amax), _p(x), _p(x_amax), _p(part), M, Cn, T, nsplit, _stream()),
                      "bm_clip_scores_h2")
            elif family == "h2_grouped":
                check(L.bm_gemm_nt_h2_grouped(_p(a), a_strides[0], a_strides[1], _p(a_amax), _p(x), x_strides[0],
                                              x_strides[1], _p(x_amax), _p(_opt(order, "order", torch.int32)),
                                              _p(_opt(seg, "seg", torch.int32)), _p(part), S, G, M, Cn, T, nsplit,
                                              _stream()), "bm_gemm_nt_h2_grouped")
            elif family == "h2_rows":
                check(L.bm_gemm_nt_h2_rows(_p(a), a_strides[0], a_strides[1], _p(a_amax), _p(a_rows), _p(x),
                                           x_strides[0], x_strides[1], _p(x_amax), _p(part), S, M, Cn, T, KS, dil,
                                           nsplit, _stream()), "bm_gemm_nt_h2")
            else:
                check(L.bm_gemm_nt_h2(_p(a), a_strides[0], a_strides[1], _p(a_amax), _p(x), x_strides[0],
                                      x_strides[1], _p(x_amax), _p(part), S, M, Cn, T, KS, dil, nsplit, _stream()),
                      "bm_gemm_nt_h2")
    _timed(label.format(_NT_SUFFIX.get(family, "_h2w")), 2.0 * S * T * M * Cn * KS, launch)


def gemm_nt(a: torch.Tensor, x: torch.Tensor, S: int, M: int, Cn: int, T: int, KS: int = 1,
            dil: int = 1, a_strides=None, x_strides=None, order=None, seg=None, G: int = 1,
            out: tp.Optional[torch.Tensor] = None, out_strides=None, nsplit: tp.Optional[int] = None):
    _req(a, "gemm_nt.a")
    _req(x, "gemm_nt.x")
    if a_strides is None:
        a_strides = (M * T, T)
    if x_strides is None:
        x_strides = (Cn * T, T)
    if out_strides is None:
        out_strides = (M * Cn * KS, Cn * KS, KS, 1)
    if out is None:
        out = torch.empty(G, M, Cn, KS, device=a.device, dtype=torch.float32)
    else:
        _touched(out)
    grouped = order is not None or seg is not None
    family, swapped, nsplit = _nt_plan(M, Cn, KS, S, T, G, dil, grouped, a_strides, x_strides, nsplit)
    if swapped:
        a, x, M, Cn, a_strides, x_strides = x, a, Cn, M, x_strides, a_strides
        out_strides = (out_strides[0], out_strides[2], out_strides[1], out_strides[3])
    canonical = tuple(out_strides) == (M * Cn * KS, Cn * KS, KS, 1)
    if nsplit == 1 and canonical:
        part = out
    else:
        part = torch.empty(G * nsplit * M * Cn * KS, device=a.device, dtype=torch.float32)
    _nt_launch(family, f"gemm_nt{{}}_kernel<KS={KS}>", a, x, part, S, G, M, Cn, T, KS, dil, a_strides, x_strides,
               order, seg, nsplit)
    if part is not out:
        check(lib().bm_reduce_splits(_p(part), _p(out), G, nsplit, M, Cn, KS, *out_strides,
                                     _stream()), "bm_reduce_splits")
    return out


class _DirectArmed:
    depth = 0

    @property
    def on(self):
        return self.depth > 0


_direct_armed = _DirectArmed()


class direct_grads_armed:

    def __enter__(self):
        _direct_armed.depth += 1
        return self

    def __exit__(self, *exc):
        _direct_armed.depth -= 1
        return False


def grad_destination(param: torch.Tensor) -> tp.Optional[torch.Tensor]:
    dst = getattr(param, "_bm_grad_dst", None)
    if dst is None or dst[1][0] or param.grad is not None or not _direct_armed.on:
        return None
    dst[1][0] = True
    return dst[0]


def gemm_nt_partials(a, x, S, M, Cn, T, a_strides, x_strides, nsplit=None):
    _req(a, "gemm_nt.a")
    _req(x, "gemm_nt.x")
    family, _, nsplit = _nt_plan(M, Cn, 1, S, T, 1, 1, False, a_strides, x_strides, nsplit, partials=True)
    part = torch.empty(nsplit, M, Cn, device=a.device, dtype=torch.float32)
    _nt_launch(family, "clip_scores:gemm_nt{}", a, x, part, S, 1, M, Cn, T, 1, 1, a_strides, x_strides, None, None, nsplit)
    return part


def sum_over_batch(x: torch.Tensor) -> torch.Tensor:
    _req(x, "sum_over_batch.x")
    B = x.shape[0]
    out = torch.empty(x.shape[1:], device=x.device, dtype=torch.float32)
    check(lib().bm_sum_over_batch(_p(x), _p(out), B, out.numel(), _stream()), "bm_sum_over_batch")
    return out


def bn_finalize(stats, count: int, gamma, beta, running_mean, running_var, num_batches,
                momentum: float, eps: float):
    _req(stats, "bn_finalize.stats")
    channel_major = getattr(stats, "_bm_channel_major", False)
    (C, ntiles, _) = stats.shape if channel_major else (stats.shape[1], stats.shape[0], 2)
    mean, invstd, scale, shift = (torch.empty(C, device=stats.device, dtype=torch.float32)
                                  for _ in range(4))
    check((lib().bm_bn_finalize_cm if channel_major else lib().bm_bn_finalize)(_p(stats), ntiles, C, count, _p(_opt(gamma, "gamma")),
                               _p(_opt(beta, "beta")), _p(_opt(running_mean, "running_mean")),
                               _p(_opt(running_var, "running_var")),
                               _p(_opt(num_batches, "num_batches", torch.int64)), momentum, eps,
                               _p(mean), _p(invstd), _p(scale), _p(shift), _stream()),
          "bm_bn_finalize")
    return mean, invstd, scale, shift


def bn_eval_affine(gamma, beta, running_mean, running_var, eps: float):
    _req(running_mean, "running_mean")
    C = running_mean.numel()
    mean, invstd, scale, shift = (torch.empty(C, device=running_mean.device, dtype=torch.float32)
                                  for _ in range(4))
    check(lib().bm_bn_eval_affine(C, _p(_opt(gamma, "gamma")), _p(_opt(beta, "beta")),
                                  _p(running_mean), _p(_req(running_var, "running_var")), eps,
                                  _p(mean), _p(invstd), _p(scale), _p(shift), _stream()),
          "bm_bn_eval_affine")
    return mean, invstd, scale, shift


def affine_act_res(y, scale, shift, res, act: int, leak: float = 0.):
    _req(y, "affine_act_res.y")
    B, C, T = y.shape
    out = torch.empty_like(y)
    check(lib().bm_affine_act_res(_p(y), _p(_opt(scale, "scale")), _p(_opt(shift, "shift")),
                                  _p(_opt(res, "res")), _p(out), B, C, T, act, leak, *_slot_args(_amax_slot(out)),
                                  _stream()), "bm_affine_act_res")
    return out


# ... 1162 lines not shown
```

### brainmagick_amd/models/common.py

```python
from functools import partial
import math
import typing as tp

import torch
from torch import nn

from .. import functional as BF
from .. import hip_ops as H


class ScaledEmbedding(nn.Module):
    def __init__(self, num_embeddings: int, embedding_dim: int, scale: float = 10.):
        super().__init__()
        self.embedding = nn.Embedding(num_embeddings, embedding_dim)
        self.embedding.weight.data /= scale
        self.scale = scale

    @property
    def weight(self):
        return self.embedding.weight * self.scale

    def forward(self, x):
        return self.embedding(x) * self.scale


class SubjectLayers(nn.Module):
    def __init__(self, in_channels: int, out_channels: int, n_subjects: int, init_id: bool = False):
        super().__init__()
        self.weights = nn.Parameter(torch.randn(n_subjects, in_channels, out_channels))
        if init_id:
            assert in_channels == out_channels
            self.weights.data[:] = torch.eye(in_channels)[None]
        self.weights.data *= 1 / in_channels**0.5

    def forward(self, x, subjects):
        return BF.SubjectLayersFn.apply(x, self.weights, subjects)

    def __repr__(self):
        S, C, D = self.weights.shape
        return f"SubjectLayers({C}, {D}, {S})"


class _Activation(nn.Module):
    def __init__(self, kind: str, leak: float = 0.):
        super().__init__()
        self.kind = kind
        self.leak = leak

    @property
    def code(self) -> int:
        return BF.ACT_CODES[self.kind]

    def extra_repr(self):
        return self.kind + (f", {self.leak}" if self.kind == "leaky" else "")


def make_activation(gelu: bool, relu_leakiness: float) -> tp.Callable[[], _Activation]:
    if gelu:
        return partial(_Activation, "gelu")
    if relu_leakiness:
        return partial(_Activation, "leaky", relu_leakiness)
    return partial(_Activation, "relu")


class _GLU(nn.Module):
    """Marker for nn.GLU(dim=1) (fused in GLUConvFn)."""


class LayerScale(nn.Module):
    def __init__(self, channels: int, init: float = 0.1, boost: float = 5.):
        super().__init__()
        self.scale = nn.Parameter(torch.zeros(channels, requires_grad=True))
        self.scale.data[:] = init / boost
        self.boost = boost

    def forward(self, x):
        return (self.boost * self.scale[:, None]) * x


class ConvSequence(nn.Module):

    def __init__(self, channels: tp.Sequence[int], kernel: int = 4, dilation_growth: int = 1,
                 dilation_period: tp.Optional[int] = None, stride: int = 2,
                 dropout: float = 0.0, leakiness: float = 0.0, groups: int = 1,
                 decode: bool = False, batch_norm: bool = False, dropout_input: float = 0,
                 skip: bool = False, scale: tp.Optional[float] = None, rewrite: bool = False,
                 activation_on_last: bool = True, post_skip: bool = False, glu: int = 0,
                 glu_context: int = 0, glu_glu: bool = True, activation: tp.Any = None) -> None:
        super().__init__()
        dilation = 1
        channels = tuple(channels)
        self.skip = skip
        self.sequence = nn.ModuleList()
        self.glus = nn.ModuleList()
        if activation is None:
            activation = partial(_Activation, "leaky", leakiness)
        self._plan: tp.List[dict] = []
        Conv = nn.Conv1d if not decode else nn.ConvTranspose1d
        strided = stride != 1 or kernel % 2 != 1 or decode
        for k, (chin, chout) in enumerate(zip(channels[:-1], channels[1:])):
            layers: tp.List[nn.Module] = []
            is_last = k == len(channels) - 2
            plan = dict(dilation=1, act=None, bn=None, glu=None, pre=None, post=[])
            if dilation_growth > 1:
                assert kernel % 2 != 0, "Supports only odd kernel with dilation for now"
            if k == 0 and dropout_input:
                assert 0 < dropout_input < 1
                layers.append(nn.Dropout(dropout_input))
                plan["pre"] = layers[-1]
            if dilation_period and (k % dilation_period) == 0:
                dilation = 1
            pad = kernel // 2 * dilation
            layers.append(Conv(chin, chout, kernel, stride, pad, dilation=dilation, groups=groups if k > 0 else 1))
            plan["conv"] = layers[-1]
            plan["dilation"] = dilation
            plan["strided"] = (stride, pad, decode) if strided else None
            dilation *= dilation_growth
            if activation_on_last or not is_last:
                if batch_norm:
                    layers.append(nn.BatchNorm1d(num_features=chout))
                    plan["bn"] = layers[-1]
                act = activation()
                layers.append(act)
                plan["act"] = act
                if dropout:
                    layers.append(nn.Dropout(dropout))
                    plan["post"].append(("dropout", layers[-1]))
                if rewrite:
                    layers += [nn.Conv1d(chout, chout, 1), _Activation("leaky", leakiness)]
                    plan["post"].append(("rewrite", layers[-2], layers[-1]))
            if chin == chout and skip:
                if scale is not None:
                    layers.append(LayerScale(chout, scale))
                    plan["post"].append(("scale", layers[-1]))
                if post_skip:
                    layers.append(Conv(chout, chout, 1, groups=chout, bias=False))
                    plan["post"].append(("post_skip", layers[-1]))
            self.sequence.append(nn.Sequential(*layers))
            if glu and (k + 1) % glu == 0:
                ch = 2 * chout if glu_glu else chout
                act = _GLU() if glu_glu else activation()
                self.glus.append(
                    nn.Sequential(
                        nn.Conv1d(chout, ch, 1 + 2 * glu_context, padding=glu_context), act))
                plan["glu"] = act
            else:
                self.glus.append(None)
            self._plan.append(plan)

    def _conv_layer(self, x, plan, code, leak, fused_residual):
        conv, bn = plan["conv"], plan["bn"]
        stride, pad, decode = plan["strided"] or (1, None, False)
        G = conv.groups
        cin, cout = conv.in_channels // G, conv.out_channels // G
        outs = []
        count0 = bn.num_batches_tracked.clone() if bn is not None and G > 1 else None
        for g in range(G):
            if G == 1:
                xg, w, b, sl = x, conv.weight, conv.bias, None
            else:
                xg = x[:, g * cin:(g + 1) * cin].contiguous()
                w = conv.weight[g * cin:(g + 1) * cin] if decode else conv.weight[g * cout:(g + 1) * cout]
                b = conv.bias[g * cout:(g + 1) * cout] if conv.bias is not None else None
                sl = slice(g * cout, (g + 1) * cout)
            if bn is not None:
                bnp = (bn.weight, bn.bias, bn.running_mean, bn.running_var) if sl is None else \
                    (bn.weight[sl], bn.bias[sl], bn.running_mean[sl], bn.running_var[sl])
                count = bn.num_batches_tracked if g == G - 1 else count0.clone()
                outs.append(BF.ConvBNActFn.apply(
                    xg, w, b, *bnp, count, self.training, plan["dilation"], code, leak, fused_residual, bn.momentum,
                    bn.eps, stride, pad, decode))
            else:
                outs.append(BF.Conv1dFn.apply(xg, w, b, plan["dilation"], code, leak, decode, stride, pad))
        return outs[0] if G == 1 else torch.cat(outs, dim=1)

    def forward(self, x: tp.Any) -> tp.Any:
        for module_idx, module in enumerate(self.sequence):
            plan = self._plan[module_idx]
            conv = plan["conv"]
            act = plan["act"]
            code = act.code if act is not None else H.ACT_NONE
            leak = act.leak if act is not None else 0.
            residual = self.skip and conv.in_channels == conv.out_channels
            old_x = x
            if plan["pre"] is not None:
                x = plan["pre"](x)
            fused_residual = residual and not plan["post"] and plan["pre"] is None and plan["strided"] is None
            x = self._conv_layer(x, plan, code, leak, fused_residual)
            for op in plan["post"]:
                if op[0] == "dropout":
                    x = op[1](x)
                elif op[0] == "rewrite":
                    x = BF.Conv1dFn.apply(x, op[1].weight, op[1].bias, 1, op[2].code, op[2].leak, False)
                elif op[0] == "scale":
                    x = op[1](x)
                else:
                    x = x * op[1].weight.view(1, -1, 1)
            if plan["strided"] is not None:
                residual = self.skip and x.shape == old_x.shape
            if residual and not (fused_residual and plan["bn"] is not None):
                x = _AddFn.apply(x if x.is_contiguous() else x.contiguous(), old_x)
            glu = self.glus[module_idx]
            if glu is not None:
                gconv = glu[0]
                if isinstance(glu[1], _GLU):
                    x = BF.GLUConvFn.apply(x, gconv.weight, gconv.bias)
                else:
                    x = BF.Conv1dFn.apply(x, gconv.weight, gconv.bias, 1, glu[1].code, glu[1].leak,
                                          False)
        return x


class _AddFn(torch.autograd.Function):
    @staticmethod
    def forward(ctx, y, res):
        return H.affine_act_res(y.contiguous(), None, None, res.contiguous(), H.ACT_NONE)

    @staticmethod
    def backward(ctx, dout):
        return dout, dout


class PositionGetter:
    INVALID = -0.1

    def __init__(self) -> None:
        self._cache: tp.Dict[int, torch.Tensor] = {}
        self._invalid_names: tp.Set[str] = set()
        self._device_cache: tp.Dict[tp.Any, tp.Tuple[torch.Tensor, torch.Tensor]] = {}
        self._layout_set_cache: tp.Dict[tp.Any, torch.Tensor] = {}
        self._layout_ids: tp.Dict[int, int] = {}
        self._layout_bytes: tp.Dict[bytes, int] = {}

    def get_recording_layout(self, recording) -> torch.Tensor:
        index = recording.recording_index
        if index in self._cache:
            return self._cache[index]
        if getattr(recording, "layout", None) is not None:
            positions = torch.as_tensor(recording.layout, dtype=torch.float32)
        else:
            positions = self._layout_from_mne(recording.mne_info)
        self._cache[index] = positions
        return positions

    def _layout_from_mne(self, info) -> torch.Tensor:
        import mne
        layout = mne.find_layout(info)
        slot_of = {name: k for k, name in enumerate(layout.names)}
        found = [(ch, slot_of[name.rsplit("-", 1)[0]]) for ch, name in enumerate(info.ch_names)
                 if name.rsplit("-", 1)[0] in slot_of]
        self._invalid_names.update(name.rsplit("-", 1)[0] for name in info.ch_names
                                   if name.rsplit("-", 1)[0] not in slot_of)
        positions = torch.full((len(info.ch_names), 2), self.INVALID)
        if found:
            channels, slots = zip(*found)
            xy = torch.as_tensor(layout.pos[list(slots), :2], dtype=torch.float64)
            lo, hi = xy.min(0).values, xy.max(0).values
            positions[list(channels)] = ((xy - lo) / (hi - lo)).float()
        return positions

    def get_positions(self, batch):
        meg = batch.meg
        B, C, T = meg.shape
        positions = torch.full((B, C, 2), self.INVALID, device=meg.device)
        for idx in range(len(batch)):
            rec_pos = self.get_recording_layout(batch._recordings[idx])
            positions[idx, :len(rec_pos)] = rec_pos.to(meg.device)
        return positions

    def get_unique_layouts(self, batch, n_channels: int, device):
        rec_ids = tuple(batch._recordings[i].recording_index for i in range(len(batch)))
        key = (rec_ids, n_channels, str(device))
        hit = self._device_cache.get(key)
        if hit is not None:
            return hit
        slots: tp.Dict[int, int] = {}
        first: tp.List[int] = []
        index: tp.List[int] = []
        for idx, rec_id in enumerate(rec_ids):
            rec_key = self._layout_ids.get(rec_id)
            if rec_key is None:
                raw = self.get_recording_layout(batch._recordings[idx]).contiguous().numpy().tobytes()
                rec_key = self._layout_ids[rec_id] = self._layout_bytes.setdefault(raw, len(self._layout_bytes))
            slot = slots.get(rec_key)
            if slot is None:
                slot = slots[rec_key] = len(first)
                first.append(idx)
            index.append(slot)
        set_key = (tuple(slots), n_channels, str(device))
        positions_u = self._layout_set_cache.get(set_key)
        if positions_u is None:
            rows = []
            for idx in first:
                pos = torch.full((n_channels, 2), self.INVALID)
                rec_pos = self.get_recording_layout(batch._recordings[idx])
                pos[:len(rec_pos)] = rec_pos
                rows.append(pos)
            positions_u = torch.stack(rows).to(device)
            if len(self._layout_set_cache) >= 64:
                self._layout_set_cache.pop(next(iter(self._layout_set_cache)))
            self._layout_set_cache[set_key] = positions_u
        layout_index = torch.tensor(index, dtype=torch.int64)
        if torch.device(device).type == "cuda":
            layout_index = layout_index.pin_memory().to(device, non_blocking=True)
        else:
            layout_index = layout_index.to(device)
        if len(self._device_cache) >= 64:
            self._device_cache.pop(next(iter(self._device_cache)))
        self._device_cache[key] = (positions_u, layout_index)
        return positions_u, layout_index

    def is_invalid(self, positions):
        return (positions == self.INVALID).all(dim=-1)


class FourierEmb(nn.Module):
    def __init__(self, dimension: int = 256, margin: float = 0.2):
        super().__init__()
        n_freqs = (dimension // 2)**0.5
        assert int(n_freqs ** 2 * 2) == dimension
        self.dimension = dimension
        self.margin = margin

    def forward(self, positions):
        return H.fourier_emb(positions.contiguous(), self.dimension, self.margin)


class ChannelDropout(nn.Module):

    N_TESTS = 100

    def __init__(self, dropout: float = 0.1, rescale: bool = True):
        super().__init__()
        self.dropout = dropout
        self.rescale = rescale
        self.position_getter = PositionGetter()
        self.ban_center_override: tp.Optional[torch.Tensor] = None

    def _centers(self, n: int, device) -> torch.Tensor:
        if self.ban_center_override is not None:
            return self.ban_center_override.to(device, torch.float32).view(1, 2).expand(n, 2)
        return torch.rand(n, 2, device=device)

    def forward(self, meg, batch):
        if not self.dropout:
            return meg
        B, C, T = meg.shape
        positions_u, layout_index = self.position_getter.get_unique_layouts(batch, C, meg.device)
        valid_u = (~self.position_getter.is_invalid(positions_u)).float()
        factor_u = valid_u
        if self.training:
            kept = ((positions_u - self._centers(1, meg.device)[0]).norm(dim=-1) > self.dropout).float()
            factor_u = factor_u * kept
            if self.rescale:
                centers = self._centers(self.N_TESTS, meg.device)
                dist = (positions_u[None] - centers[:, None, None, :]).norm(dim=-1)
                proba_kept = torch.zeros_like(valid_u)
                for n in range(self.N_TESTS):
                    proba_kept += (dist[n] > self.dropout).float() / self.N_TESTS
                factor_u = factor_u / (1e-8 + proba_kept)
        return meg * factor_u[layout_index][:, :, None]


class ChannelMerger(nn.Module):
    def __init__(self, chout: int, pos_dim: int = 256,
                 dropout: float = 0, usage_penalty: float = 0.,
                 n_subjects: int = 200, per_subject: bool = False):
        super().__init__()
        assert pos_dim % 4 == 0
        self.position_getter = PositionGetter()
        self.per_subject = per_subject
        if self.per_subject:
            self.heads = nn.Parameter(torch.randn(n_subjects, chout, pos_dim, requires_grad=True))
        else:
            self.heads = nn.Parameter(torch.randn(chout, pos_dim, requires_grad=True))
        self.heads.data /= pos_dim ** 0.5
        self.dropout = dropout
        self.embedding = FourierEmb(pos_dim)
        self.usage_penalty = usage_penalty
        self._penalty = torch.tensor(0.)
        self.ban_center_override: tp.Optional[torch.Tensor] = None

    @property
    def training_penalty(self):
        return self._penalty.to(next(self.parameters()).device)

    def layouts_and_ban(self, meg, batch):
        B, C, T = meg.shape
        positions_u, layout_index = self.position_getter.get_unique_layouts(batch, C, meg.device)
        ban_center, radius = None, 0.
        if self.training and self.usage_penalty > 0.:
            self._penalty = torch.tensor(float(self.usage_penalty))
        if self.training and self.dropout:
            if self.ban_center_override is not None:
                ban_center = self.ban_center_override.to(meg.device, torch.float32)
            else:
                ban_center = torch.rand(2, device=meg.device)
            radius = float(self.dropout)
        return positions_u, layout_index, ban_center, radius

    def forward(self, meg, batch):
        positions_u, layout_index, ban_center, radius = self.layouts_and_ban(meg, batch)
        if self.per_subject:
            n_subjects = self.heads.shape[0]
            subjects = BF.H.index_i32(batch.subject_index.to(meg.device, torch.int64).contiguous(),
                                      n_subjects).to(torch.int64)
            pairs, inverse = torch.unique(layout_index * n_subjects + subjects, return_inverse=True)
            return BF.ChannelMergerFn.apply(meg, self.heads[pairs % n_subjects].contiguous(),
                                            positions_u[pairs // n_subjects].contiguous(), inverse.contiguous(),
                                            ban_center, radius)
        return BF.ChannelMergerFn.apply(meg, self.heads, positions_u, layout_index, ban_center,
                                        radius)


def pad_multiple(x: torch.Tensor, base: int):
    length = x.shape[-1]
    target = math.ceil(length / base) * base
    return torch.nn.functional.pad(x, (0, target - length))


class DualPathRNN(nn.Module):

    def __init__(self, channels: int, depth: int, inner_length: int = 10):
        super().__init__()
        self.lstms = nn.ModuleList([nn.LSTM(channels, channels, 1) for _ in range(depth * 4)])
        self.inner_length = inner_length

    def forward(self, x: torch.Tensor) -> torch.Tensor:
        length = x.shape[-1]
        seq = pad_multiple(x, self.inner_length).permute(2, 0, 1).contiguous()
        steps, batch, channels = seq.shape
        chunks = steps // self.inner_length
        vendor_rnn = torch.backends.cudnn.enabled
        torch.backends.cudnn.enabled = False
        try:
            for k, lstm in enumerate(self.lstms):
                out = lstm(seq)[0]
                if k % 2 == 0:
                    out = out.view(self.inner_length, chunks, batch, channels).transpose(0, 1) \
                        .reshape(steps, batch, channels)
                seq = seq + out
                if k % 2 == 1:
                    seq = seq.flip(0)
        finally:
            torch.backends.cudnn.enabled = vendor_rnn
        return seq[:length].permute(1, 2, 0).contiguous()
```

### brainmagick_amd/models/simpleconv.py

```python
import random
import typing as tp

import torch
from torch import nn

from .common import (
    ConvSequence, ScaledEmbedding, SubjectLayers, ChannelMerger, ChannelDropout, DualPathRNN, make_activation)
from .. import functional as BF
from .. import hip_ops as H


_FUSE_FRONT_END = True


class SimpleConv(nn.Module):

    def __init__(self, in_channels: tp.Dict[str, int], out_channels: int, hidden: tp.Dict[str, int],
                 depth: int = 4, concatenate: bool = False, linear_out: bool = False,
                 complex_out: bool = False, kernel_size: int = 5, growth: float = 1.,
                 dilation_growth: int = 2, dilation_period: tp.Optional[int] = None, skip: bool = False,
                 post_skip: bool = False, scale: tp.Optional[float] = None, rewrite: bool = False,
                 groups: int = 1, glu: int = 0, glu_context: int = 0, glu_glu: bool = True,
                 gelu: bool = False, dual_path: int = 0, conv_dropout: float = 0.0,
                 dropout_input: float = 0.0, batch_norm: bool = False, relu_leakiness: float = 0.0,
                 n_subjects: int = 200, subject_dim: int = 64, subject_layers: bool = False,
                 subject_layers_dim: str = "input", subject_layers_id: bool = False,
                 embedding_scale: float = 1.0, n_fft: tp.Optional[int] = None, fft_complex: bool = True,
                 merger: bool = False, merger_pos_dim: int = 256, merger_channels: int = 270,
                 merger_dropout: float = 0.2, merger_penalty: float = 0., merger_per_subject: bool = False,
                 dropout: float = 0., dropout_rescale: bool = True, initial_linear: int = 0,
                 initial_depth: int = 1, initial_nonlin: bool = False, subsample_meg_channels: int = 0):
        super().__init__()
        if set(in_channels) != set(hidden):
            raise ValueError("Channels and hidden keys must match "
                             f"({set(in_channels.keys())} and {set(hidden.keys())})")
        if n_fft is not None:
            raise NotImplementedError(
                "SimpleConv option n_fft (torchaudio STFT front end) is outside the MI355X hot path: no grid of the "
                "paper uses it (SURVEY.md §2.2), and torchaudio being absent from this image the reference itself "
                "cannot run it here, so there would be nothing to hold an implementation to")
        if "meg" not in in_channels:
            raise ValueError("SimpleConv needs a 'meg' input (the sensor front end is built around it)")
        if kernel_size % 2 != 1:
            raise AssertionError("For padding to work, this must be verified")
        if linear_out and complex_out:
            raise AssertionError("linear_out and complex_out are exclusive")
        self.out_channels = out_channels
        self._concatenate = concatenate
        activation = make_activation(gelu, relu_leakiness)
        in_channels, hidden = dict(in_channels), dict(hidden)

        width = in_channels["meg"]
        self.dropout = ChannelDropout(dropout, dropout_rescale) if dropout > 0. else None
        self.subsampled_meg_channels: tp.Optional[list] = None
        if subsample_meg_channels:
            self._subsample(width, subsample_meg_channels)
        width = self._build_front_end(
            width, activation, hidden["meg"], n_subjects,
            merger=dict(on=merger, channels=merger_channels, pos_dim=merger_pos_dim, dropout=merger_dropout,
                        penalty=merger_penalty, per_subject=merger_per_subject),
            linear=dict(width=initial_linear, depth=initial_depth, nonlin=initial_nonlin),
            subject=dict(layers=subject_layers, where=subject_layers_dim, init_id=subject_layers_id,
                         emb_dim=subject_dim, emb_scale=embedding_scale))

        in_channels["meg"] = width
        if concatenate:
            in_channels = {"concat": sum(in_channels.values())}
            hidden = {"concat": sum(hidden.values())}
        widths = {name: [in_channels[name]] + [int(round(hidden[name] * growth ** k)) for k in range(depth)]
                  for name in in_channels}
        stack_kw = dict(kernel=kernel_size, stride=1, leakiness=relu_leakiness, dropout=conv_dropout,
                        dropout_input=dropout_input, batch_norm=batch_norm, dilation_growth=dilation_growth,
                        groups=groups, dilation_period=dilation_period, skip=skip, post_skip=post_skip,
                        scale=scale, rewrite=rewrite, glu=glu, glu_context=glu_context, glu_glu=glu_glu,
                        activation=activation)
        top = sum(w[-1] for w in widths.values())
        self.dual_path = DualPathRNN(top, dual_path) if dual_path else None
        if linear_out:
            self.final = nn.ConvTranspose1d(top, out_channels, 1, 1, 0)
        elif complex_out:
            self.final = nn.Sequential(nn.Conv1d(top, 2 * top, 1), activation(),
                                       nn.ConvTranspose1d(2 * top, out_channels, 1, 1, 0))
        else:
            assert len(widths) == 1, "if no linear_out, there must be a single branch."
            self.final = None
            stack_kw["activation_on_last"] = False
            next(iter(widths.values()))[-1] = out_channels
        self.encoders = nn.ModuleDict({name: ConvSequence(w, **stack_kw) for name, w in widths.items()})

    def _subsample(self, n_sensors: int, keep_n: int):
        order = list(range(n_sensors))
        random.Random(1234).shuffle(order)
        self.subsampled_meg_channels = order[:keep_n]
        keep = torch.zeros(1, n_sensors, 1)
        keep[:, self.subsampled_meg_channels] = 1.
        self.register_buffer("_channel_keep", keep, persistent=False)

    def _build_front_end(self, width: int, activation, hidden: int, n_subjects: int, merger: dict,
                         linear: dict, subject: dict) -> int:
        self.merger = self.initial_linear = self.subject_layers = self.subject_embedding = None
        if merger["on"]:
            self.merger = ChannelMerger(merger["channels"], pos_dim=merger["pos_dim"], dropout=merger["dropout"],
                                        usage_penalty=merger["penalty"], n_subjects=n_subjects,
                                        per_subject=merger["per_subject"])
            width = merger["channels"]
        if linear["width"]:
            layers: tp.List[nn.Module] = [nn.Conv1d(width, linear["width"], 1)]
            for _ in range(linear["depth"] - 1):
                layers += [activation(), nn.Conv1d(linear["width"], linear["width"], 1)]
            if linear["nonlin"]:
                layers.append(activation())
            self.initial_linear = nn.Sequential(*layers)
            width = linear["width"]
        if subject["layers"]:
            out = {"hidden": hidden, "input": width}[subject["where"]]
            self.subject_layers = SubjectLayers(width, out, n_subjects, subject["init_id"])
            width = out
        if subject["emb_dim"]:
            self.subject_embedding = ScaledEmbedding(n_subjects, subject["emb_dim"], subject["emb_scale"])
            width += subject["emb_dim"]
        return width

    def _front_end_is_linear_chain(self) -> bool:
        return (self.merger is not None and self.subject_layers is not None and self.initial_linear is not None
                and len(self.initial_linear) == 1 and self.subsampled_meg_channels is None
                and not self.merger.per_subject)

    def forward(self, inputs, batch):
        subjects = batch.subject_index
        length = next(iter(inputs.values())).shape[-1]
        x = inputs["meg"]
        if not x.is_cuda:
            raise RuntimeError("brainmagick_amd.SimpleConv runs on the MI355X HIP path only; got a "
                               f"{x.device} tensor (there is no CPU fallback)")
        if x.dtype != torch.float32:
            raise TypeError(f"SimpleConv expects fp32 inputs like the reference, got {x.dtype}")

        if self.subsampled_meg_channels is not None:
            x = x * self._channel_keep
        if self.dropout is not None:
            x = self.dropout(x, batch)
        fused = self._front_end_is_linear_chain() and _FUSE_FRONT_END
        if fused:
            positions_u, layout_index, ban_center, radius = self.merger.layouts_and_ban(x, batch)
            fused = positions_u.shape[0] * self.subject_layers.weights.shape[0] <= x.shape[0]
        self.front_end_fused = fused
        if fused:
            conv = self.initial_linear[0]
            x = BF.FusedFrontEndFn.apply(x, self.merger.heads, conv.weight, conv.bias, self.subject_layers.weights,
                                         positions_u, layout_index, subjects, ban_center, radius)
        elif self.merger is not None and self._front_end_is_linear_chain() and _FUSE_FRONT_END:
            x = BF.ChannelMergerFn.apply(x, self.merger.heads, positions_u, layout_index, ban_center, radius)
        elif self.merger is not None:
            x = self.merger(x, batch)
        if fused:
            pass
        elif self.initial_linear is not None:
            mods = list(self.initial_linear)
            i = 0
            while i < len(mods):
                conv = mods[i]
                act = mods[i + 1] if i + 1 < len(mods) and not isinstance(mods[i + 1], nn.Conv1d) \
                    else None
                x = BF.Conv1dFn.apply(x, conv.weight, conv.bias, 1,
                                      act.code if act is not None else H.ACT_NONE,
                                      act.leak if act is not None else 0., False)
                i += 2 if act is not None else 1
        if self.subject_layers is not None and not fused:
            x = self.subject_layers(x, subjects)
        if self.subject_embedding is not None:
            emb = self.subject_embedding(subjects)[:, :, None]
            x = torch.cat([x, emb.expand(-1, -1, length)], dim=1)
        inputs["meg"] = x

        if self._concatenate:
            x = self.encoders["concat"](torch.cat([v for _, v in sorted(inputs.items())], dim=1))
        elif len(self.encoders) == 1:
            x = self.encoders["meg"](x)
        else:
            x = torch.cat([self.encoders[name](v) for name, v in sorted(inputs.items())], dim=1)
        if self.dual_path is not None:
            x = self.dual_path(x)
        if self.final is not None:
            if isinstance(self.final, nn.ConvTranspose1d):
                x = BF.Conv1dFn.apply(x, self.final.weight, self.final.bias, 1, H.ACT_NONE, 0., True)
            else:
                conv, act, tconv = self.final[0], self.final[1], self.final[2]
                x = BF.Conv1dFn.apply(x, conv.weight, conv.bias, 1, act.code, act.leak, False)
                x = BF.Conv1dFn.apply(x, tconv.weight, tconv.bias, 1, H.ACT_NONE, 0., True)
        assert x.shape[-1] >= length
        return x if x.shape[-1] == length else x[:, :, :length]
```

### include/bm_hip.h

```cpp
#ifndef BM_HIP_H
#define BM_HIP_H
#ifdef __cplusplus
extern "C" {
#endif

#define BM_ACT_NONE 0
#define BM_ACT_GELU 1
#define BM_ACT_RELU 2
#define BM_ACT_LEAKY 3

int bm_version(void);
const char* bm_last_error(void);
int bm_device_count(void);

int bm_conv_mt_for(int M);
int bm_conv_mpad(int M);
int bm_conv_stats_tiles(int B, int T);
long bm_packed_weight_elems(int G, int M, int Cin, int KS);
int bm_pack_weights(const float* src, float* dst, int G, int M, int Cin, int KS, long sg, long sm,
                    long sc, long sj, int flip, const float* alpha_ptr, void* stream);
int bm_group_by_index(const long* idx, int B, int G, int* order, int* seg, int* err_flag, void* stream);
int bm_index_to_i32(const long* idx, int B, int G, int* out, int* err_flag, void* stream);
int bm_reduce_splits(const float* part, float* out, int G, int nsplit, int M, int Cn, int KS, long sg,
                     long sm, long sc, long sj, void* stream);
int bm_sum_over_batch(const float* x, float* out, int B, long n, void* stream);

int bm_conv1d_nn(const float* x, long x_bstride, const float* wpacked, const int* widx,
                 const float* bias, long bias_gstride, const float* ep_scale, const float* ep_shift, const float* res,
                 long res_bstride, float* y_pre, float* y_out, long y_bstride, float* stats, int B,
                 int Cin, int M, int T, int KS, int dil, int act, float leak, void* stream);

int bm_conv1d_out_len(int T, int KS, int stride, int dil, int pad, int transposed);
int bm_conv_strided_stats_tiles(int B, int Tout, int stride, int transposed);
int bm_conv1d_strided(const float* x, long x_bstride, const float* wpacked, const float* bias,
                      const float* ep_scale, const float* ep_shift, float* y_pre, float* y_out, long y_bstride,
                      float* stats, int B, int Cin, int M, int T, int Tout, int KS, int stride, int dil, int pad,
                      int act, float leak, void* stream);
int bm_conv1d_transposed(const float* x, long x_bstride, const float* wpacked, const float* bias,
                         const float* ep_scale, const float* ep_shift, float* y_pre, float* y_out, long y_bstride,
                         float* stats, int B, int Cin, int M, int T, int Tout, int KS, int stride, int dil, int pad,
                         int act, float leak, void* stream);
int bm_conv1d_strided_wgrad_suggest_splits(int R, int Q, int KS, int S, int U);
int bm_conv1d_strided_wgrad(const float* a, long a_sstride, const float* xl, long xl_sstride, float* part, int S,
                            int R, int Q, int U, int L, int KS, int stride, int dil, int pad, int nsplit,
                            void* stream);

int bm_lstm_layer_fwd(const float* whh0, const float* whh1, const float* gx0, const float* gx1, float* y,
                      float* gates0, float* gates1, float* c0, float* c1, int H, int B, int T, int dirs,
                      void* stream);
int bm_lstm_layer_bwd(const float* whh0, const float* whh1, const float* dy, const float* gates0,
                      const float* gates1, const float* c0, const float* c1, float* dg0, float* dg1,
                      float* dc0, float* dc1, int H, int B, int T, int dirs, void* stream);

long bm_packed_weight_elems_x3(int G, int M, int Cin, int KS);
int bm_pack_weights_x3(const float* src, void* dst, int G, int M, int Cin, int KS, long sg, long sm,
                       long sc, long sj, int flip, const float* alpha_ptr, void* stream);
int bm_conv1d_nn_x3(const float* x, long x_bstride, const void* wpacked, const int* widx,
                    const float* bias, long bias_gstride, const float* ep_scale, const float* ep_shift, const float* res,
                    long res_bstride, float* y_pre, float* y_out, long y_bstride, float* stats, int B,
                    int Cin, int M, int T, int KS, int dil, int act, float leak, void* stream);
int bm_gemm_nt_x3(const float* a, long a_sstride, long a_rstride, const float* x, long x_sstride,
                  long x_rstride, const int* order, const int* seg, float* part, int S, int G, int M,
                  int Cn, int T, int KS, int dil, int nsplit, void* stream);
int bm_conv_x3_mt_for(int M);
int bm_conv_x3_mpad(int M);

int bm_conv_h2_mw_for(int M);
int bm_conv_h2_mpad(int M);
int bm_conv_h2_covers(int Cin, int M, int T, int KS, int dil);
long bm_packed_weight_bytes_h2(int G, int M, int Cin, int KS);
int bm_pack_weights_h2(const float* src, void* dst, int G, int M, int Cin, int KS, long sg, long sm, long sc,
                       long sj, int flip, const float* alpha_ptr, void* stream);
int bm_pack_h2_job_bytes(void);
int bm_pack_h2_job_fill(void* job, const float* src, void* dst, int G, int M, int Cin, int KS, long sg, long sm,
                        long sc, long sj, int flip, const float* alpha_ptr, int block0);
int bm_pack_weights_h2_batch(const void* jobs_dev, int njobs, int total_blocks, int max_nk, void* stream);
int bm_amax_ws_elems(void);
int bm_amax(const float* x, long n, float* out, float* amax_ws, void* stream);
int bm_amax_checked(const float* x, long n, float* out, float* amax_ws, int* nonfinite_flag, void* stream);
int bm_conv_h2_stats_tiles(int B, int T);
int bm_conv1d_nn_h2(const float* x, long x_bstride, const float* x_amax, const void* wpacked, const int* widx,
                    const float* bias, long bias_gstride, const float* ep_scale, const float* ep_shift, const float* res,
                    long res_bstride, float* y_pre, float* y_out, long y_bstride, float* stats, int B, int Cin,
                    int M, int T, int KS, int dil, int act, float leak, int G, float* y_amax_out, float* amax_ws,
                    void* stream);

int bm_gemm_nt_h2_covers(int M, int Cn, int KS, int S, int T, int G, int dil, int ordered);
int bm_gemm_nt_h2_suggest_splits(int M, int Cn, int KS, int S, int T);
int bm_gemm_nt_h2(const float* a, long a_sstride, long a_rstride, const float* a_amax, const float* x,
                  long x_sstride, long x_rstride, const float* x_amax, float* part, int S, int M, int Cn, int T,
                  int KS, int dil, int nsplit, void* stream);
int bm_gemm_nt_h2_rows(const float* a, long a_sstride, long a_rstride, const float* a_amax, const float* a_row_amax,
                       const float* x, long x_sstride, long x_rstride, const float* x_amax, float* part, int S,
                       int M, int Cn, int T, int KS, int dil, int nsplit, void* stream);

int bm_gemm_nt_h2_grouped(const float* a, long a_sstride, long a_rstride, const float* a_amax, const float* x,
                          long x_sstride, long x_rstride, const float* x_amax, const int* order, const int* seg,
                          float* part, int S, int G, int M, int Cn, int T, int nsplit, void* stream);
int bm_gemm_nt_h2_suggest_splits_grouped(int M, int Cn, int KS, int S, int T, int G);

int bm_clip_scores_h2_covers(int B, int Bc, long K);
int bm_clip_scores_h2_suggest_splits(int B, int Bc, long K);
int bm_clip_scores_h2(const float* est, const float* est_amax, const float* cand, const float* cand_amax, float* part,
                      int B, int Bc, long K, int nsplit, void* stream);

int bm_gemm_nt_suggest_splits(int M, int Cn, int KS, int S, int T, int G);
int bm_clip_suggest_splits(int M, int Cn, int S, int T);
int bm_gemm_nt(const float* a, long a_sstride, long a_rstride, const float* x, long x_sstride,
               long x_rstride, const int* order, const int* seg, float* part, int S, int G, int M,
               int Cn, int T, int KS, int dil, int nsplit, void* stream);

int bm_bn_finalize(const float* stats, int ntiles, int C, long count, const float* gamma,
                   const float* beta, float* running_mean, float* running_var, long* num_batches,
                   float momentum, float eps, float* mean, float* invstd, float* scale, float* shift,
                   void* stream);
int bm_bn_finalize_cm(const float* stats, int ntiles, int C, long count, const float* gamma,
                   const float* beta, float* running_mean, float* running_var, long* num_batches,
                   float momentum, float eps, float* mean, float* invstd, float* scale, float* shift,
                   void* stream);
int bm_bn_eval_affine(int C, const float* gamma, const float* beta, const float* running_mean,
                      const float* running_var, float eps, float* mean, float* invstd, float* scale,
                      float* shift, void* stream);
int bm_affine_act_res(const float* y, const float* scale, const float* shift, const float* res,
                      float* out, int B, int C, int T, int act, float leak, float* amax_out, float* amax_ws,
                      void* stream);
int bm_bwd_nsplit(int B);
long bm_act_bn_bwd_workspace_bytes(int B, int C);
int bm_act_bn_bwd_set_fused(int mode);
int bm_act_bn_bwd_set_poll_limit(int polls);
long bm_act_bn_bwd_fused_fallbacks(void);
int bm_act_bn_bwd_fused_covers(int B, int C, int T);
int bm_act_bn_bwd(const float* dout, const float* y, const float* scale, const float* shift,
                  const float* mean, const float* invstd, int bn_train, float* dy, float* dgamma,
                  float* dbeta, float* dbias, void* workspace, long workspace_bytes, int B, int C,
                  int T, int act, float leak, float* amax_out, float* amax_ws, float* amax_rows_out,
                  void* stream);
long bm_channel_sum_workspace_bytes(int B, int C);
int bm_channel_sum(const float* x, long bstride, float* out, void* workspace, long workspace_bytes,
                   int B, int C, int T, void* stream);
int bm_channel_stats_splits(int B);
int bm_channel_stats(const float* x, float* stats, int B, int C, int T, void* stream);
int bm_glu_fwd(const float* u, float* out, int B, int H, int T, float* amax_out, float* amax_ws, void* stream);
long bm_glu_bwd_workspace_bytes(int B, int H);
int bm_glu_bwd(const float* dout, const float* u, float* du, float* dbias, void* workspace,
               long workspace_bytes, int B, int H, int T, float* amax_out, float* amax_ws,
               float* amax_rows_out, void* stream);
int bm_time_sums_t(const float* x, float* out, int B, int C, int T, void* stream);

int bm_center_scale(const float* x, float* out, const long* group, const float* center,
                    const float* scale, int B, int C, int T, int clip, float limit, float* maxabs,
                    void* stream);

long bm_quantile_select_workspace_bytes(int C, int Q);
int bm_quantile_select(const float* x, const long* ranks, float* out, int N, int C, int T, int Q, void* workspace,
                       long workspace_bytes, void* stream);
long bm_masked_moments_workspace_bytes(int channels);
int bm_masked_moments(const float* x, const unsigned char* mask, int mask_mode, int N, int F, int T, int f0, int f1,
                      int per_channel, float* mean, float* std, double* count, void* workspace, long workspace_bytes,
                      void* stream);
long bm_category_counts_workspace_bytes(int cardinality);
int bm_category_counts(const float* x, const unsigned char* mask, int mask_mode, int N, int F, int T, int f,
                       int cardinality, float* counts, int* flags, void* workspace, long workspace_bytes, void* stream);
int bm_center_scale_inverse(const float* x, float* out, const long* group, const float* center, const float* scale,
                            int B, int C, int T, void* stream);

int bm_fourier_emb(const float* positions, float* emb, long rows, int D, float margin, void* stream);
int bm_masked_softmax(const float* scores, const float* positions, const float* ban_center,
                      float ban_radius, float* weights, int U, int O, int C, void* stream);
int bm_softmax_bwd(const float* w, const float* dw, float* ds, long rows, int C, void* stream);

int bm_clip_inv_norms(const float* cand, int Bc, long K, float* inv_norm, void* stream);
int bm_clip_cand_prep(const float* cand, int Bc, long K, float* inv_norm, float* amax_slot, int* nonfinite_flag,
                      void* stream);
int bm_flag_unless_all_set(const unsigned char* mask, long n, int* flag, void* stream);
int bm_clip_ce(const float* part, int nsplit, const float* inv_norm, float* scores, float* probs,
               float* dscaled, float* loss_row, float* loss, int B, int Bc, int target_offset,
               void* stream);
int bm_clip_ce_masked(const float* part, int nsplit, const float* inv_norm, const float* col_valid, float* scores,
                      float* probs, float* dscaled, float* loss_row, float* loss, int B, int Bc, int target_offset,
                      void* stream);

int bm_clip_ce_cols(const float* scores, const float* inv_norm, float* dscaled, float* loss_col, float* loss, int B,
                    int Bc, int target_offset, float w_row, float w_col, void* stream);

long bm_regress_workspace_bytes(void);
int bm_regress_loss_fwd(const float* est, const float* out, const unsigned char* mask, int mask_mode, int B, int F,
                        int T, int kind, float* loss, double* count, void* workspace, long workspace_bytes, int* flag,
                        void* stream);
int bm_regress_loss_bwd(const float* est, const float* out, const unsigned char* mask, int mask_mode, int B, int F,
                        int T, int kind, const float* grad_out, const double* count, float* d_est, float* d_out,
                        float* amax_out, float* amax_rows_out, void* workspace, long workspace_bytes, void* stream);
int bm_regress_metric_update(const float* est, long est_bstride, const float* out, long out_bstride,
                             const unsigned char* mask, long mask_bstride, int mask_full, int B, int F, int T, int t0,
                             double* acc, void* stream);

long bm_meg_init_workspace_bytes(void);
int bm_meg_init(const float* meg, float* x, int B, int C, int T, int limit, float* amax_out, void* workspace,
                long workspace_bytes, void* stream);

long bm_lowpass_workspace_bytes(void);
int bm_lowpass(const float* x, long row_stride, float* y, int rows, int T, int keep, const float* taps, int half,
               float* amax_out, void* workspace, long workspace_bytes, void* stream);

long bm_spectral_table_entry_bytes(void);
long bm_spectral_ws_floats(int rows, int cols, int niters);
long bm_spectral_ws_doubles(int rows, int cols, int niters);
int bm_spectral_table_fill(void* entry, const float* w, int rows, int cols, long ld, int dim, long r_off,
                           long ws_float_off, long ws_double_off, long grad_off);
int bm_spectral_fwd(const void* table, int nmat, int max_slabs, const float* R, int dim, int niters,
                    float* ws_floats, double* ws_doubles, float* values, float* total, void* stream);
int bm_spectral_bwd(const void* table, int nmat, int max_slabs, int max_tiles, int niters, float* ws_floats,
                    double* ws_doubles, const float* gscale, float* grads, void* stream);

long bm_segment_table_entry_bytes(void);
int bm_segment_table_fill(void* entry, const void* base, long n, int rows);
int bm_segment_gather(const void* table, int R, const int* rec, const int* start, long n_index, long first, int B, int C,
                      int T, int base0, int base1, int elem_bytes, void* dst, int* flag, void* stream);

long bm_features_table_entry_bytes(int which);
int bm_features_kind_fill(void* entry, const double* start, const double* dur, const double* runmax, long n);
int bm_features_source_fill(void* entry, const void* data);
int bm_features_array_fill(void* entry, const float* base, long L, double er);
int bm_segment_features(const int* feat_table, const float* feat_default, int NF, int NK, int mask_kind,
                        const void* kinds, const void* srcs, int R, const int* rec, const double* wstart,
                        const double* wdur, long n_index, long first, int B, int F, int T, double sr, float* dst,
                        unsigned char* mask, int* flag, void* stream);

long bm_wave_table_entry_bytes(void);
int bm_wave_table_fill(void* entry, const float* x, long L, float* out);

int bm_mel_frame_tile(int n_fft);
int bm_wave_moments_splits(long L);
int bm_wave_moments(const void* table, const long* lengths, int n_waves, unsigned* tickets, double* part,
                    int max_splits, double* mom, void* stream);
int bm_mel_spectrogram(const void* table, const long* lengths, int n_waves, const double* mom, const float* basis,
                       int n_fft, int nbp, const float* fbw, const int* range, const int* range_host, int n_mels,
                       int use_log, float eps, void* stream);

int bm_resample_frames_tile(int old_rate, int new_rate, int width);
int bm_resample_frac(const void* table, const long* lengths, int n_waves, const double* mom, const float* taps,
                     int old_rate, int new_rate, int width, void* stream);

int bm_yin_frames_tile(void);
int bm_yin_pitch(const void* table, const long* lengths, int n_waves, double sr, int w_len, int w_step, int tau_min,
                 int tau_max, double thresh, void* stream);

int bm_feature_decoding_fwd(const float* est, const float* out, const unsigned char* mask, const float* weights,
                            long n_weights, const int* table, int n_features, int B, int C, int Co, int T, float* loss,
                            float* terms, double* denoms, float* lse, void* workspace, long workspace_bytes, int* flag,
                            void* stream);
int bm_feature_decoding_bwd(const float* est, const float* out, const unsigned char* mask, const float* weights,
                            long n_weights, const int* table, int n_features, int B, int C, int Co, int T,
                            const float* grad_out, const double* denoms, const float* lse, float* d_est, void* stream);
int bm_class_acc_update(const float* est, long est_bstride, const float* target, long target_bstride,
                        const unsigned char* mask, long mask_bstride, int B, int K, int T, int t0, long* acc,
                        void* stream);

int bm_clip_cand_coef(const float* dscaled, const float* scores, const float* inv_norm,
                      const float* alpha, float* coef, int B, int Bc, void* stream);
int bm_row_axpy_sub(float* y, const float* x, const float* coef, int rows, long K, void* stream);
int bm_topk_rows(const float* x, int rows, int cols, int k, int* idx_out, float* val_out,
                 const long* col_labels, const long* row_labels, int* hit_out, void* stream);

int bm_row_softmax(const float* x, float* y, int rows, int cols, void* stream);
int bm_rowwise_dot(const float* a, const float* b, const float* scale, float* out, int rows, long K,
                   void* stream);
int bm_segment_sum_cols(const float* p, const int* order, const int* seg, float* pv, int rows, int cols,
                        int V, void* stream);

int bm_adam_step(float* param, const float* grad, float* exp_avg, float* exp_avg_sq, long n, int step,
                 double lr, double beta1, double beta2, double eps, double grad_scale, void* stream);

int bm_comm_unique_id_bytes(void);
int bm_comm_available(void);
int bm_comm_unique_id(void* out_id);
int bm_comm_init(const void* id, int world, int rank, int device, void** handle);
int bm_comm_destroy(void* handle);
int bm_comm_world(void* handle);
int bm_comm_rank(void* handle);
int bm_comm_reported_world(void* handle);
int bm_comm_reported_rank(void* handle);
int bm_comm_allgather(void* handle, const float* send, float* recv, long count, void* stream);
int bm_comm_reduce_scatter(void* handle, const float* send, float* recv, long count, void* stream);
int bm_comm_allreduce(void* handle, const float* send, float* recv, long count, int op, void* stream);

#ifdef __cplusplus
}
#endif
#endif
```

Measured before the change: 17300 segments/s.

## Fuse GLU and activation backward into consumer conv backward-data epilogue

Adds an 'input-op' variant of the f16x2 conv kernel whose epilogue applies the backward of the preceding GLU (with the residual add) or of the preceding activation. It writes the resulting gradients directly and emits per-row sum/max pairs, which a fold kernel reduces into amax and row sums. The models now skip the separate GLU/activation in forward when the next conv can own it, so the standalone elementwise backward kernels and their extra memory passes go away. The cost is a heavier epilogue with more buffer loads and registers, plus extra plumbing across the autograd functions.

```diff
diff --git a/brainmagick_amd/csrc/bm_common.h b/brainmagick_amd/csrc/bm_common.h
--- a/brainmagick_amd/csrc/bm_common.h
+++ b/brainmagick_amd/csrc/bm_common.h
@@ -144,6 +144,8 @@
 int bm_amax_finalize_rows(const float* ws, int C, int nsplit, float* out, float* rows_out, hipStream_t stream);
 int bm_amax_finalize_rows_sums(const float* ws, int C, int nsplit, float* out, float* rows_out,
                                const double* sum_partial, float* sums_out, hipStream_t stream);
+int bm_pair_fold(const float* pairs, int rows, int ntl, const float* ws, int nparts, float* out, float* rows_out,
+                 float* sums_out, hipStream_t stream);
 static inline BmAmaxDst bm_amax_dst(float* amax_out, float* amax_ws) {
     return BmAmaxDst{amax_out ? amax_ws : nullptr};
 }
diff --git a/brainmagick_amd/csrc/conv_h2_common.h b/brainmagick_amd/csrc/conv_h2_common.h
--- a/brainmagick_amd/csrc/conv_h2_common.h
+++ b/brainmagick_amd/csrc/conv_h2_common.h
@@ -16,7 +16,14 @@
     const float* x_amax;
     const float* wscale;
     BmAmaxDst y_amax;
+    const float* aux;
+    long aux_bstride;
+    float* pairs;
+    int aux_act;
+    float aux_leak;
 };
+
+enum { H2EP_PLAIN = 0, H2EP_RES = 1, H2EP_RES_GLUBWD = 2, H2EP_ACTBWD = 3 };
 
 template <int MW>
 struct H2Simple {
@@ -183,7 +190,155 @@
     });
 }
 
-template <int MW, bool RESK = false>
+__device__ __forceinline__ int h2_fold_sum_max(float (&s)[16], float (&m)[16], int lane) {
+    const bool b4 = lane & 16, b3 = lane & 8, b2 = lane & 4, b1 = lane & 2;
+#define H2_FOLD(N_, BIT_, MASK_)                                                                  \
+    _Pragma("unroll") for (int i = 0; i < N_; ++i) {                                              \
+        const float k1 = BIT_ ? s[i + N_] : s[i], g1 = BIT_ ? s[i] : s[i + N_];                    \
+        const float k2 = BIT_ ? m[i + N_] : m[i], g2 = BIT_ ? m[i] : m[i + N_];                    \
+        s[i] = k1 + __shfl_xor(g1, MASK_);                                                        \
+        m[i] = fmaxf(k2, __shfl_xor(g2, MASK_));                                                  \
+    }
+    H2_FOLD(8, b4, 16)
+    H2_FOLD(4, b3, 8)
+    H2_FOLD(2, b2, 4)
+    H2_FOLD(1, b1, 2)
+#undef H2_FOLD
+    s[0] += __shfl_xor(s[0], 1);
+    m[0] = fmaxf(m[0], __shfl_xor(m[0], 1));
+    const int q = (b4 ? 8 : 0) + (b3 ? 4 : 0) + (b2 ? 2 : 0) + (b1 ? 1 : 0);
+    return (q & 3) + 8 * (q >> 2);
+}
+
+struct H2Walk {
+    int voff;
+    int rowb;
+    int tb;
+    int row0, M;
+    const float* fl;
+    const float* bl;
+    bool cok[3];
+};
+__device__ __forceinline__ float h2_buf_ld(__amdgpu_buffer_rsrc_t r, int off) {
+    return __builtin_bit_cast(float, __builtin_amdgcn_raw_buffer_load_b32(r, off, 0, 0));
+}
+__device__ __forceinline__ void h2_buf_st(float v, __amdgpu_buffer_rsrc_t r, int off) {
+    __builtin_amdgcn_raw_buffer_store_b32(__builtin_bit_cast(unsigned, v), r, off, 0, 0);
+}
+#define H2_WALK_OFF(W_, MT_, NT_, R_) ((W_).voff + (W_).rowb + ((MT_) * 32 + ((R_) & 3) + 8 * ((R_) >> 2)) * (W_).tb + (NT_) * 128)
+
+template <int MW>
+__device__ __forceinline__ float h2_act_bwd_tile(const H2Walk& w, f32x16 (&acc)[MW][3], __amdgpu_buffer_rsrc_t auxr,
+                                                 __amdgpu_buffer_rsrc_t yr, int act, float leak, float* pairs_tile,
+                                                 long row_stride, int lane) {
+    constexpr int NBLK = MW * 3, D = 4;
+    float zv[D][16];
+    float s[16], m[16];
+    float amx = 0.f;
+    bm_static_for<NBLK + D>([&](auto ic) __attribute__((always_inline)) {
+        constexpr int i = decltype(ic)::value;
+        if constexpr (i >= D) {
+            constexpr int b = i - D, mt = b / 3, nt = b % 3;
+            if constexpr (nt == 0) {
+#pragma unroll
+                for (int r = 0; r < 16; ++r) s[r] = m[r] = 0.f;
+            }
+            if (w.cok[nt]) {
+#pragma unroll
+                for (int r = 0; r < 16; ++r) {
+                    const int rl = mt * 32 + (r & 3) + 8 * (r >> 2);
+                    const float d = fmaf(acc[mt][nt][r], w.fl[rl], w.bl[rl]);
+                    const float z = zv[b % D][r];
+                    float g;
+                    if (act == BM_ACT_GELU_FASTGRAD) g = bm_gelu_grad_fast(z);
+                    else g = act == BM_ACT_RELU ? (!(z <= 0.f) ? 1.f : 0.f) : act == BM_ACT_LEAKY ? (z > 0.f ? 1.f : leak) : 1.f;
+                    const float y = d * g;
+                    h2_buf_st(y, yr, H2_WALK_OFF(w, mt, nt, r));
+                    s[r] += y;
+                    m[r] = fmaxf(m[r], fabsf(y));
+                }
+            }
+            if constexpr (nt == 2) {
+                const int row = w.row0 + mt * 32 + h2_fold_sum_max(s, m, lane);
+                if (row < w.M) amx = fmaxf(amx, m[0]);
+                if (!(lane & 1) && row < w.M) *reinterpret_cast<float2*>(pairs_tile + (long)row * row_stride) = float2{s[0], m[0]};
+            }
+        }
+        if constexpr (i < NBLK) {
+            constexpr int mt = i / 3, nt = i % 3;
+            if (w.cok[nt]) {
+#pragma unroll
+                for (int r = 0; r < 16; ++r) zv[i % D][r] = h2_buf_ld(auxr, H2_WALK_OFF(w, mt, nt, r));
+            }
+        }
+        __builtin_amdgcn_sched_barrier(0);
+    });
+    return amx;
+}
+
+template <int MW>
+__device__ __forceinline__ float h2_glu_bwd_tile(const H2Walk& w, f32x16 (&acc)[MW][3], __amdgpu_buffer_rsrc_t resr,
+                                                 __amdgpu_buffer_rsrc_t ua, __amdgpu_buffer_rsrc_t ug,
+                                                 __amdgpu_buffer_rsrc_t ya, __amdgpu_buffer_rsrc_t yg, float* pairs_tile,
+                                                 long row_stride, int lane) {
+    constexpr int NBLK = MW * 3, D = 2;
+    float rv[D][16], av[D][16], gv[D][16];
+    float sa[16], ma[16], sg[16], mg[16];
+    float amx = 0.f;
+    bm_static_for<NBLK + D>([&](auto ic) __attribute__((always_inline)) {
+        constexpr int i = decltype(ic)::value;
+        if constexpr (i >= D) {
+            constexpr int b = i - D, mt = b / 3, nt = b % 3;
+            if constexpr (nt == 0) {
+#pragma unroll
+                for (int r = 0; r < 16; ++r) sa[r] = ma[r] = sg[r] = mg[r] = 0.f;
+            }
+            if (w.cok[nt]) {
+#pragma unroll
+                for (int r = 0; r < 16; ++r) {
+                    const int rl = mt * 32 + (r & 3) + 8 * (r >> 2);
+                    const float d = fmaf(acc[mt][nt][r], w.fl[rl], w.bl[rl]) + rv[b % D][r];
+                    const float a = av[b % D][r], g = gv[b % D][r];
+                    const float sgm = 1.f / (1.f + expf(-g));
+                    const float oa = d * sgm;
+                    const float og = d * a * sgm * (1.f - sgm);
+                    const int off = H2_WALK_OFF(w, mt, nt, r);
+                    h2_buf_st(oa, ya, off);
+                    h2_buf_st(og, yg, off);
+                    sa[r] += oa;
+                    sg[r] += og;
+                    ma[r] = fmaxf(ma[r], fabsf(oa));
+                    mg[r] = fmaxf(mg[r], fabsf(og));
+                }
+            }
+            if constexpr (nt == 2) {
+                const int row = w.row0 + mt * 32 + h2_fold_sum_max(sa, ma, lane);
+                h2_fold_sum_max(sg, mg, lane);
+                if (row < w.M) amx = fmaxf(amx, fmaxf(ma[0], mg[0]));
+                if (!(lane & 1) && row < w.M) {
+                    *reinterpret_cast<float2*>(pairs_tile + (long)row * row_stride) = float2{sa[0], ma[0]};
+                    *reinterpret_cast<float2*>(pairs_tile + (long)(w.M + row) * row_stride) = float2{sg[0], mg[0]};
+                }
+            }
+        }
+        if constexpr (i < NBLK) {
+            constexpr int mt = i / 3, nt = i % 3;
+            if (w.cok[nt]) {
+#pragma unroll
+                for (int r = 0; r < 16; ++r) {
+                    const int off = H2_WALK_OFF(w, mt, nt, r);
+                    rv[i % D][r] = h2_buf_ld(resr, off);
+                    av[i % D][r] = h2_buf_ld(ua, off);
+                    gv[i % D][r] = h2_buf_ld(ug, off);
+                }
+            }
+        }
+        __builtin_amdgcn_sched_barrier(0);
+    });
+    return amx;
+}
+
+template <int MW, int EP = H2EP_PLAIN>
 __device__ __forceinline__ void h2_tile_epilogue(const ConvH2Args& args, f32x16 (&acc)[MW][3], float* smem, int b, int g,
                                                  int m0, int n0, int ntile, float sx_inv, int tid, int lane, int wm,
                                                  int wn, int nl, int h, unsigned* trace_out = nullptr) {
@@ -205,7 +360,7 @@
     }
     __syncthreads();
     H2_TE(1)
-    if constexpr (RESK) {
+    if constexpr (EP == H2EP_RES) {
         const float* fl = ep + 3 * HBM + wm * (MW * 32) + 4 * h;
         const float* bl = ep + wm * (MW * 32) + 4 * h;
 #pragma unroll
@@ -233,6 +388,36 @@
         } else {
             h2_residual_add<MW, false>(e, acc, col0, a.T);
             amx = h2_plain_tile<MW, false>(e, acc, col0, a.T);
+        }
+        bm_publish_amax(amx, args.y_amax, smem + 4 * HBM);
+        return;
+    }
+    if constexpr (EP == H2EP_RES_GLUBWD || EP == H2EP_ACTBWD) {
+        H2Walk w;
+        w.voff = ((4 * h) * a.T + n0 + wn * (NW * 32) + nl) * 4;
+        w.rowb = (m0 + wm * (MW * 32)) * a.T * 4;
+        w.tb = a.T * 4;
+        w.row0 = m0 + wm * (MW * 32) + 4 * h;
+        w.M = a.M;
+        w.fl = ep + 3 * HBM + wm * (MW * 32) + 4 * h;
+        w.bl = ep + wm * (MW * 32) + 4 * h;
+        const int col0 = n0 + wn * (NW * 32) + nl;
+        w.cok[0] = col0 < a.T; w.cok[1] = col0 + 32 < a.T; w.cok[2] = col0 + 64 < a.T;
+        float* pt = args.pairs + (long)((b * a.ntiles_n + ntile) * 2 + wn) * 2;
+        const long prs = (long)a.B * a.ntiles_n * 4;
+        const unsigned seg = (unsigned)(a.M * a.T * 4);
+        float amx;
+        if constexpr (EP == H2EP_ACTBWD) {
+            amx = h2_act_bwd_tile<MW>(w, acc, bm_buffer_rsrc(args.aux + (long)b * args.aux_bstride, seg),
+                                      bm_buffer_rsrc(a.y_out + (long)b * a.y_bstride, seg), args.aux_act, args.aux_leak,
+                                      pt, prs, lane);
+        } else {
+            const float* ub = args.aux + (long)b * args.aux_bstride;
+            float* yb = a.y_out + (long)b * a.y_bstride;
+            const long goff = (long)a.M * a.T;
+            amx = h2_glu_bwd_tile<MW>(w, acc, bm_buffer_rsrc(a.res + (long)b * a.res_bstride, seg), bm_buffer_rsrc(ub, seg),
+                                      bm_buffer_rsrc(ub + goff, seg), bm_buffer_rsrc(yb, seg), bm_buffer_rsrc(yb + goff, seg),
+                                      pt, prs, lane);
         }
         bm_publish_amax(amx, args.y_amax, smem + 4 * HBM);
         return;
diff --git a/brainmagick_amd/csrc/conv_nn_h2w.hip b/brainmagick_amd/csrc/conv_nn_h2w.hip
--- a/brainmagick_amd/csrc/conv_nn_h2w.hip
+++ b/brainmagick_amd/csrc/conv_nn_h2w.hip
@@ -47,8 +47,8 @@
     return H2RItem{H2R_BREAD, i};
 }
 
-template <int KS, int MW, bool RESK = false>
-__global__ __launch_bounds__(256, 1) void conv_nn_h2w_kernel(ConvH2Args args) {
+template <int KS, int MW, int EP>
+__device__ __forceinline__ void conv_nn_h2w_tile(const ConvH2Args& args) {
     const ConvNNArgs& a = args.c;
 #ifdef HG_TRACE
     const unsigned t_kernel0 = (unsigned)__builtin_readcyclecounter();
@@ -206,9 +206,9 @@
 #undef H2R_LOAD_X
 
 #ifdef HG_TRACE
-    h2_tile_epilogue<MW, RESK>(args, acc, smem, b, g, m0, n0, ntile, sx_inv, tid, lane, wm, wn, nl, h, ch_trace_buf);
+    h2_tile_epilogue<MW, EP>(args, acc, smem, b, g, m0, n0, ntile, sx_inv, tid, lane, wm, wn, nl, h, ch_trace_buf);
 #else
-    h2_tile_epilogue<MW, RESK>(args, acc, smem, b, g, m0, n0, ntile, sx_inv, tid, lane, wm, wn, nl, h);
+    h2_tile_epilogue<MW, EP>(args, acc, smem, b, g, m0, n0, ntile, sx_inv, tid, lane, wm, wn, nl, h);
 #endif
 #ifdef HG_TRACE
     asm volatile("s_waitcnt vmcnt(0)" ::: "memory");
@@ -219,6 +219,16 @@
         o[8 + 5] = t_loop1 - t_loop0;
     }
 #endif
+}
+
+template <int KS, int MW, bool RESK = false>
+__global__ __launch_bounds__(256, 1) void conv_nn_h2w_kernel(ConvH2Args args) {
+    conv_nn_h2w_tile<KS, MW, RESK ? H2EP_RES : H2EP_PLAIN>(args);
+}
+template <int KS, int MW, int EP>
+__global__ __launch_bounds__(256, 1) void conv_h2w_inop_kernel(ConvH2Args args) {
+    static_assert(EP == H2EP_RES_GLUBWD || EP == H2EP_ACTBWD, "the other kinds are conv_nn_h2w_kernel");
+    conv_nn_h2w_tile<KS, MW, EP>(args);
 }
 
 extern "C" int bm_conv_h2_mw_for(int M) {
@@ -281,7 +291,7 @@
     BM_REQUIRE(G >= 1, "conv1d_nn_h2: bad dims");
     BM_REQUIRE(!stats || (y_pre && !y_out && !ep_scale && act == BM_ACT_NONE && !res),
                "conv1d_nn_h2: per-tile statistics come with y_pre alone (the training-mode BatchNorm layers)");
-    ConvH2Args args;
+    ConvH2Args args{};
     ConvNNArgs& a = args.c;
     if (int e = conv_nn_fill_args(a, "conv1d_nn_h2", x, x_bstride, (const float*)wpacked, widx, bias, bias_gstride, ep_scale,
                                   ep_shift, res, res_bstride, y_pre, y_out, y_bstride, stats, B, Cin, M, T, KS, dil, act,
@@ -308,3 +318,72 @@
     }
 #undef H2_DISPATCH
 }
+
+extern "C" int bm_conv_h2_inop_covers(int B, int Cin, int M, int T, int KS, int dil, int kind) {
+    if (kind != 1 && kind != 2) return 0;
+    if (KS != (kind == 1 ? 1 : 3) || B < 1 || Cin < 1 || M < 1 || T < 1 || dil < 1) return 0;
+    if (!bm_conv_h2_covers(Cin, M, T, KS, dil)) return 0;
+    if ((long)bm_conv_h2_mpad(M) * T * 4 >= 0x7fffffffL) return 0;
+    const long nblocks = (long)B * cdiv(T, HBN) * (bm_conv_h2_mpad(M) / (64 * bm_conv_h2_mw_for(M)));
+    return nblocks <= BM_AMAX_WS;
+}
+
+template <int KS, int MW, int EP>
+static int launch_conv_h2w_inop(ConvH2Args args, int rows, float* y_amax_out, float* amax_rows_out, float* sums_out,
+                                hipStream_t stream) {
+    constexpr int HBM = 64 * MW;
+    const size_t lds_ep = (size_t)(4 * HBM + 4) * sizeof(float);
+    const size_t lds = (size_t)(2 * HXSLAB) * 16 > lds_ep ? (size_t)(2 * HXSLAB) * 16 : lds_ep;
+    args.c.ntiles_n = cdiv(args.c.T, HBN);
+    args.c.ntiles_m = args.c.Mpad / HBM;
+    const long nblocks = (long)args.c.B * args.c.ntiles_n * args.c.ntiles_m;
+    if (nblocks <= 0) return BM_OK;
+    hipLaunchKernelGGL((conv_h2w_inop_kernel<KS, MW, EP>), dim3((unsigned)nblocks), dim3(256), lds, stream, args);
+    if (int rc = bm_check_launch("conv_h2w_inop")) return rc;
+    return bm_pair_fold(args.pairs, rows, bm_conv_h2_stats_tiles(args.c.B, args.c.T), args.y_amax.ws, (int)nblocks,
+                        y_amax_out, amax_rows_out, sums_out, stream);
+}
+
+extern "C" int bm_conv1d_nn_h2_inop(const float* x, long x_bstride, const float* x_amax, const void* wpacked,
+                                    const float* bias, const float* res, long res_bstride, const float* aux,
+                                    long aux_bstride, float* y, long y_bstride, float* pairs, int B, int Cin, int M,
+                                    int T, int KS, int dil, int kind, int act, float leak, float* y_amax_out,
+                                    float* amax_ws, float* amax_rows_out, float* sums_out, void* stream) {
+    BM_REQUIRE(x_amax && aux && y && pairs, "conv1d_nn_h2_inop: null pointer");
+    BM_REQUIRE(y_amax_out && amax_ws && amax_rows_out && sums_out, "conv1d_nn_h2_inop: the side outputs are not optional");
+    BM_REQUIRE(kind == 1 || kind == 2, "conv1d_nn_h2_inop: kind is 1 (act backward) or 2 (residual + GLU backward)");
+    BM_REQUIRE((kind == 2) == (res != nullptr), "conv1d_nn_h2_inop: the residual comes with kind 2, and only with it");
+    BM_REQUIRE(act == BM_ACT_NONE || act == BM_ACT_GELU || act == BM_ACT_RELU || act == BM_ACT_LEAKY,
+               "conv1d_nn_h2_inop: unknown activation %d", act);
+    ConvH2Args args{};
+    ConvNNArgs& a = args.c;
+    if (int e = conv_nn_fill_args(a, "conv1d_nn_h2_inop", x, x_bstride, (const float*)wpacked, nullptr, bias, 0, nullptr,
+                                  nullptr, res, res_bstride, nullptr, y, y_bstride, nullptr, B, Cin, M, T, KS, dil,
+                                  BM_ACT_NONE, 0.f))
+        return e;
+    BM_REQUIRE(bm_conv_h2_inop_covers(B, Cin, M, T, KS, dil, kind),
+               "conv1d_nn_h2_inop: launch not covered (B=%d Cin=%d M=%d T=%d KS=%d dil=%d kind=%d)", B, Cin, M, T, KS, dil, kind);
+    const int mw = bm_conv_h2_mw_for(M);
+    a.Mpad = bm_conv_h2_mpad(M);
+    a.nchunk = cdiv(Cin, 32);
+    const long f16_elems = (long)a.nchunk * KS * 2 * 4 * a.Mpad * 8;
+    args.x_amax = x_amax;
+    args.y_amax = bm_amax_dst(y_amax_out, amax_ws);
+    args.wscale = reinterpret_cast<const float*>(reinterpret_cast<const char*>(wpacked) + f16_elems * 2);
+    args.aux = aux;
+    args.aux_bstride = aux_bstride;
+    args.pairs = pairs;
+    args.aux_act = act == BM_ACT_GELU ? BM_ACT_GELU_FASTGRAD : act;
+    args.aux_leak = leak;
+    hipStream_t s = (hipStream_t)stream;
+    const int rows = kind == 2 ? 2 * M : M;
+#define H2_INOP(MW_)                                                                                             \
+    return kind == 1 ? launch_conv_h2w_inop<1, MW_, H2EP_ACTBWD>(args, rows, y_amax_out, amax_rows_out, sums_out, s) \
+                     : launch_conv_h2w_inop<3, MW_, H2EP_RES_GLUBWD>(args, rows, y_amax_out, amax_rows_out, sums_out, s);
+    switch (mw) {
+        case 5: H2_INOP(5)
+        case 4: H2_INOP(4)
+        default: H2_INOP(2)
+    }
+#undef H2_INOP
+}
diff --git a/brainmagick_amd/csrc/core.hip b/brainmagick_amd/csrc/core.hip
--- a/brainmagick_amd/csrc/core.hip
+++ b/brainmagick_amd/csrc/core.hip
@@ -19,7 +19,7 @@
 }
 
 extern "C" const char* bm_last_error(void) { return bm_err_buf; }
-extern "C" int bm_version(void) { return 116; }
+extern "C" int bm_version(void) { return 117; }
 
 extern "C" int bm_device_count(void) {
     int n = 0;
@@ -71,4 +71,38 @@
     return bm_check_launch("amax_finalize_rows");
 }
 
+__global__ __launch_bounds__(256) void pair_fold_kernel(const float2* __restrict__ pairs, int rows, int ntl,
+                                                        const float* __restrict__ ws, int nparts, float* __restrict__ out,
+                                                        float* __restrict__ rows_out, float* __restrict__ sums_out) {
+    __shared__ float sh[4];
+    if (blockIdx.x == 0) {
+        bm_amax_fold<4>(ws, nparts, out, sh);
+        return;
+    }
+    const int r = ((int)blockIdx.x - 1) * 4 + (int)(threadIdx.x >> 6);
+    if (r >= rows) return;
+    const int lane = threadIdx.x & 63;
+    const float2* row = pairs + (long)r * ntl;
+    double s = 0;
+    float m = 0.f;
+    for (int i = lane; i < ntl; i += 64) {
+        const float2 p = row[i];
+        s += (double)p.x;
+        m = fmaxf(m, p.y);
+    }
+    s = bm_wave_sum_d(s);
+    m = bm_wave_max(m);
+    if (lane == 0) {
+        rows_out[r] = m;
+        sums_out[r] = (float)s;
+    }
+}
+
+int bm_pair_fold(const float* pairs, int rows, int ntl, const float* ws, int nparts, float* out, float* rows_out,
+                 float* sums_out, hipStream_t stream) {
+    hipLaunchKernelGGL(pair_fold_kernel, dim3(1 + cdiv(rows, 4)), dim3(256), 0, stream,
+                       reinterpret_cast<const float2*>(pairs), rows, ntl, ws, nparts, out, rows_out, sums_out);
+    return bm_check_launch("pair_fold");
+}
+
 extern "C" int bm_amax_ws_elems(void) { return BM_AMAX_WS; }
diff --git a/brainmagick_amd/functional.py b/brainmagick_amd/functional.py
--- a/brainmagick_amd/functional.py
+++ b/brainmagick_amd/functional.py
@@ -6,6 +6,8 @@
 
 
 ACT_CODES = {"none": H.ACT_NONE, "gelu": H.ACT_GELU, "relu": H.ACT_RELU, "leaky": H.ACT_LEAKY}
+
+FUSE_INPUT_OPS = True
 
 
 def _c(t: torch.Tensor) -> torch.Tensor:
@@ -67,7 +69,7 @@
     return H.conv_nn(x, wp, M, KS, dil, res=res, **kw)
 
 
-def _layer_backward(ctx, dy, x, weight, geom, res=None, publish_amax=True):
+def _layer_backward(ctx, dy, x, weight, geom, res=None, publish_amax=True, input_op=None):
     dil, transposed, stride, pad = geom
     KS = weight.shape[2]
     Cin, T = x.shape[1], x.shape[2]
@@ -89,31 +91,52 @@
                 wp = H.pack_weights(weight, 1, Cin, M, 1, 0, M, 1, 0, shape=(T, dil))
             else:
                 wp = H.pack_conv_dgrad(weight, (T, dil))
-            _, dx, _ = H.conv_nn(dy, wp, Cin, KS, dil, res=res, publish_amax=publish_amax)
+            if input_op is None:
+                _, dx, _ = H.conv_nn(dy, wp, Cin, KS, dil, res=res, publish_amax=publish_amax)
+            else:
+                dx = _input_op_backward(dy, wp, Cin, KS, dil, res, input_op)
     return dx, dw
 
 
+def _input_op_backward(dy, wp, Cin, KS, dil, res, input_op):
+    kind, aux, act, leak = input_op
+    if FUSE_INPUT_OPS and H.conv_input_op_covers(wp, dy.shape[0], dy.shape[1], Cin, dy.shape[2], KS, dil, kind):
+        return H.conv_nn_input_op(dy, wp, Cin, KS, dil, aux, kind, res=res, act=act, leak=leak)
+    _, dx, _ = H.conv_nn(dy, wp, Cin, KS, dil, res=res, publish_amax=False)
+    if kind == H.INPUT_OP_GLU:
+        daux, sums = H.glu_bwd(dx, aux, want_dbias=True)
+    else:
+        daux, _, _, sums = H.act_bn_bwd(dx, aux, None, None, None, None, False, act, leak, want_dbias=True)
+    return H.note_row_sums(daux, sums)
+
+
 class Conv1dFn(torch.autograd.Function):
 
     @staticmethod
     def forward(ctx, x, weight, bias, dil: int, act: int, leak: float, transposed_weight: bool, stride: int = 1,
-                pad=None):
+                pad=None, input_act: int = H.ACT_NONE, input_leak: float = 0., publish_out: bool = True,
+                publish_dx: bool = True):
         x, weight = _c(x), _c(weight)
         geom = (dil, transposed_weight, stride, pad)
+        aux = None
+        if input_act != H.ACT_NONE:
+            assert pad is None and act == H.ACT_NONE, "an owned input activation: \"same\" family, no activation behind"
+            aux, x = x, H.affine_act_res(x, None, None, None, input_act, input_leak)
         need_pre = act != H.ACT_NONE and any(ctx.needs_input_grad[:3])
         if need_pre and pad is None:
             pre, _, _ = _layer_forward(x, weight, geom, bias=bias, want_pre=True, want_out=False)
             out = H.affine_act_res(pre, None, None, None, act, leak)
         else:
-            pre, out, _ = _layer_forward(x, weight, geom, bias=bias, act=act, leak=leak, want_pre=need_pre)
-        ctx.save_for_backward(x, weight, pre)
-        ctx.cfg = (geom, act, leak, bias is not None)
+            kw = {} if publish_out or pad is not None else dict(publish_amax=False)
+            pre, out, _ = _layer_forward(x, weight, geom, bias=bias, act=act, leak=leak, want_pre=need_pre, **kw)
+        ctx.save_for_backward(x, weight, pre, aux)
+        ctx.cfg = (geom, act, leak, bias is not None, input_act, input_leak, publish_dx)
         return out
 
     @staticmethod
     def backward(ctx, dout):
-        x, weight, pre = ctx.saved_tensors
-        geom, act, leak, has_bias = ctx.cfg
+        x, weight, pre, aux = ctx.saved_tensors
+        geom, act, leak, has_bias, input_act, input_leak, publish_dx = ctx.cfg
         dout = _c(dout)
         dbias = None
         if act != H.ACT_NONE:
@@ -122,9 +145,12 @@
         else:
             dy = dout
             if has_bias:
-                dbias = H.channel_sum(dy)
-        dx, dw = _layer_backward(ctx, dy, x, weight, geom)
-        return (dx, dw, dbias) + (None,) * 6
+                dbias = H.row_sums_of(dy)
+                if dbias is None:
+                    dbias = H.channel_sum(dy)
+        input_op = None if aux is None else (H.INPUT_OP_ACT, aux, input_act, input_leak)
+        dx, dw = _layer_backward(ctx, dy, x, weight, geom, publish_amax=publish_dx, input_op=input_op)
+        return (dx, dw, dbias) + (None,) * 10
 
 
 class ConvBNActFn(torch.autograd.Function):
@@ -132,9 +158,13 @@
     @staticmethod
     def forward(ctx, x, weight, bias, gamma, beta, running_mean, running_var, num_batches,
                 training: bool, dil: int, act: int, leak: float, residual: bool, momentum: float,
-                eps: float, stride: int = 1, pad=None, transposed: bool = False):
+                eps: float, stride: int = 1, pad=None, transposed: bool = False, input_glu: bool = False):
         x, weight = _c(x), _c(weight)
         geom = (dil, transposed, stride, pad)
+        u = None
+        if input_glu:
+            assert pad is None and residual, "an owned input GLU: a residual layer of the \"same\" family"
+            u, x = x, H.glu_fwd(x)
         res = x if residual else None
         needs_grad = any(ctx.needs_input_grad[:5])
         if training:
@@ -146,19 +176,20 @@
             mean, invstd, scale, shift = H.bn_eval_affine(gamma, beta, running_mean, running_var, eps)
             pre, out, _ = _layer_forward(x, weight, geom, res=res, bias=bias, scale=scale, shift=shift, act=act,
                                          leak=leak, want_pre=needs_grad)
-        ctx.save_for_backward(x, weight, pre, scale, shift, mean, invstd)
+        ctx.save_for_backward(x, weight, pre, scale, shift, mean, invstd, u)
         ctx.cfg = (geom, training, act, leak, residual, bias is not None)
         return out
 
     @staticmethod
     def backward(ctx, dout):
-        x, weight, pre, scale, shift, mean, invstd = ctx.saved_tensors
+        x, weight, pre, scale, shift, mean, invstd, u = ctx.saved_tensors
         geom, training, act, leak, residual, has_bias = ctx.cfg
         dout = _c(dout)
         dy, dgamma, dbeta, dbias = H.act_bn_bwd(dout, pre, scale, shift, mean, invstd, training, act,
                                                 leak, want_affine_grads=True, want_dbias=has_bias)
-        dx, dw = _layer_backward(ctx, dy, x, weight, geom, res=dout if residual else None, publish_amax=False)
-        return (dx, dw, dbias, dgamma, dbeta) + (None,) * 13
+        dx, dw = _layer_backward(ctx, dy, x, weight, geom, res=dout if residual else None, publish_amax=False,
+                                 input_op=None if u is None else (H.INPUT_OP_GLU, u, H.ACT_NONE, 0.))
+        return (dx, dw, dbias, dgamma, dbeta) + (None,) * 14
 
 
 class GLUConvFn(torch.autograd.Function):
diff --git a/brainmagick_amd/hip_ops.py b/brainmagick_amd/hip_ops.py
--- a/brainmagick_amd/hip_ops.py
+++ b/brainmagick_amd/hip_ops.py
@@ -185,7 +185,7 @@
 
 
 def _touched(t: torch.Tensor) -> torch.Tensor:
-    for attr in ("_bm_amax", "_bm_row_amax", "_bm_inv_norms"):
+    for attr in ("_bm_amax", "_bm_row_amax", "_bm_row_sums", "_bm_inv_norms"):
         if getattr(t, attr, None) is not None:
             try:
                 delattr(t, attr)
@@ -378,6 +378,59 @@
         return f"conv_nn{_MODE_SUFFIX[mode]}_kernel<{tile}>"
     _timed(label, 2.0 * B * T * M * Cin * KS, launch)
     return y_pre, y_out, stats
+
+
+INPUT_OP_ACT, INPUT_OP_GLU = 1, 2
+
+
+def conv_input_op_covers(wpacked: torch.Tensor, B: int, Cin: int, M: int, T: int, KS: int, dil: int, kind: int) -> bool:
+    return getattr(wpacked, "_bm_mode", "") == "f16x2" and getattr(wpacked, "_bm_groups", 0) == 1 and \
+        bool(lib().bm_conv_h2_inop_covers(B, Cin, M, T, KS, dil, kind))
+
+
+def row_sums_of(t: torch.Tensor) -> tp.Optional[torch.Tensor]:
+    return _noted(t, "_bm_row_sums")
+
+
+def note_row_sums(t: torch.Tensor, sums: torch.Tensor) -> torch.Tensor:
+    _note(t, "_bm_row_sums", sums)
+    return t
+
+
+def conv_nn_input_op(x: torch.Tensor, wpacked: torch.Tensor, M: int, KS: int, dil: int, aux: torch.Tensor, kind: int,
+                     res: tp.Optional[torch.Tensor] = None, bias=None, act: int = ACT_NONE,
+                     leak: float = 0.) -> torch.Tensor:
+    _req(x, "conv_nn_input_op.x")
+    _req(aux, "conv_nn_input_op.aux")
+    _req(wpacked, "conv_nn_input_op.w", torch.uint8)
+    B, Cin, T = x.shape
+    rows = 2 * M if kind == INPUT_OP_GLU else M
+    if not conv_input_op_covers(wpacked, B, Cin, M, T, KS, dil, kind):
+        raise BmHipError(f"conv_nn_input_op: launch not covered (B={B} Cin={Cin} M={M} T={T} KS={KS} dil={dil} "
+                         f"kind={kind}, weights packed as {getattr(wpacked, '_bm_mode', 'f32')})")
+    assert aux.shape == (B, rows, T), (aux.shape, (B, rows, T))
+    if kind == INPUT_OP_GLU:
+        _req(res, "conv_nn_input_op.res")
+        assert res.shape == (B, M, T), (res.shape, (B, M, T))
+    else:
+        assert res is None
+    y = torch.empty(B, rows, T, device=x.device, dtype=torch.float32)
+    pairs = torch.empty(rows, lib().bm_conv_h2_stats_tiles(B, T), 2, device=x.device, dtype=torch.float32)
+    sums = torch.empty(rows, device=x.device, dtype=torch.float32)
+    x_amax = amax(x)
+    slot = _amax_slot(y)
+    assert slot is not None, "conv_nn_input_op runs in f16x2 mode only"
+    row_max = _row_amax_out(y, slot)
+    _note(y, "_bm_row_sums", sums)
+
+    def launch():
+        check(lib().bm_conv1d_nn_h2_inop(_p(x), Cin * T, _p(x_amax), _p(wpacked), _p(_opt(bias, "bias")), _p(res), M * T,
+                                         _p(aux), rows * T, _p(y), rows * T, _p(pairs), B, Cin, M, T, KS, dil, kind, act,
+                                         leak, *_slot_args(slot), _p(row_max), _p(sums), _stream()),
+              "bm_conv1d_nn_h2_inop")
+    _timed(lambda: f"conv_nn_h2w_kernel<{KS},{lib().bm_conv_h2_mw_for(M)}>+{'glu_bwd' if kind == INPUT_OP_GLU else 'act_bwd'}",
+           2.0 * B * T * M * Cin * KS, launch)
+    return y
 
 
 def conv_out_len(T: int, KS: int, stride: int, dil: int, pad: int, transposed: bool) -> int:
diff --git a/brainmagick_amd/models/common.py b/brainmagick_amd/models/common.py
--- a/brainmagick_amd/models/common.py
+++ b/brainmagick_amd/models/common.py
@@ -148,7 +148,7 @@
                 self.glus.append(None)
             self._plan.append(plan)
 
-    def _conv_layer(self, x, plan, code, leak, fused_residual):
+    def _conv_layer(self, x, plan, code, leak, fused_residual, input_glu=False):
         conv, bn = plan["conv"], plan["bn"]
         stride, pad, decode = plan["strided"] or (1, None, False)
         G = conv.groups
@@ -169,12 +169,26 @@
                 count = bn.num_batches_tracked if g == G - 1 else count0.clone()
                 outs.append(BF.ConvBNActFn.apply(
                     xg, w, b, *bnp, count, self.training, plan["dilation"], code, leak, fused_residual, bn.momentum,
-                    bn.eps, stride, pad, decode))
+                    bn.eps, stride, pad, decode, input_glu))
             else:
                 outs.append(BF.Conv1dFn.apply(xg, w, b, plan["dilation"], code, leak, decode, stride, pad))
         return outs[0] if G == 1 else torch.cat(outs, dim=1)
 
+    def _owns_input_glu(self, module_idx: int, x) -> bool:
+        if not BF.FUSE_INPUT_OPS or module_idx >= len(self._plan) or H.get_compute_dtype() != "f16x2":
+            return False
+        plan = self._plan[module_idx]
+        conv = plan["conv"]
+        if plan["bn"] is None or plan["post"] or plan["pre"] is not None or plan["strided"] is not None or \
+                conv.groups != 1 or not (self.skip and conv.in_channels == conv.out_channels):
+            return False
+        B, C, T = x.shape
+        KS, dil = conv.kernel_size[0], plan["dilation"]
+        return C == conv.in_channels and bool(H.lib().bm_conv_h2_covers(C, C, T, KS, dil)) and \
+            bool(H.lib().bm_conv_h2_inop_covers(B, C, C, T, KS, dil, H.INPUT_OP_GLU))
+
     def forward(self, x: tp.Any) -> tp.Any:
+        input_glu = False
         for module_idx, module in enumerate(self.sequence):
             plan = self._plan[module_idx]
             conv = plan["conv"]
@@ -186,7 +200,8 @@
             if plan["pre"] is not None:
                 x = plan["pre"](x)
             fused_residual = residual and not plan["post"] and plan["pre"] is None and plan["strided"] is None
-            x = self._conv_layer(x, plan, code, leak, fused_residual)
+            x = self._conv_layer(x, plan, code, leak, fused_residual, input_glu)
+            input_glu = False
             for op in plan["post"]:
                 if op[0] == "dropout":
                     x = op[1](x)
@@ -203,7 +218,11 @@
             glu = self.glus[module_idx]
             if glu is not None:
                 gconv = glu[0]
-                if isinstance(glu[1], _GLU):
+                if isinstance(glu[1], _GLU) and self._owns_input_glu(module_idx + 1, x):
+                    input_glu = True
+                    x = BF.Conv1dFn.apply(x, gconv.weight, gconv.bias, 1, H.ACT_NONE, 0., False, 1, None, H.ACT_NONE, 0.,
+                                          False, False)
+                elif isinstance(glu[1], _GLU):
                     x = BF.GLUConvFn.apply(x, gconv.weight, gconv.bias)
                 else:
                     x = BF.Conv1dFn.apply(x, gconv.weight, gconv.bias, 1, glu[1].code, glu[1].leak,
diff --git a/brainmagick_amd/models/simpleconv.py b/brainmagick_amd/models/simpleconv.py
--- a/brainmagick_amd/models/simpleconv.py
+++ b/brainmagick_amd/models/simpleconv.py
@@ -125,6 +125,19 @@
         return (self.merger is not None and self.subject_layers is not None and self.initial_linear is not None
                 and len(self.initial_linear) == 1 and self.subsampled_meg_channels is None
                 and not self.merger.per_subject)
+
+    @staticmethod
+    def _head_owns_activation(x, conv, tconv) -> bool:
+        if not (BF.FUSE_INPUT_OPS and torch.is_grad_enabled() and H.get_compute_dtype() == "f16x2"):
+            return False
+        if conv.kernel_size[0] != 1 or tconv.kernel_size[0] != 1:
+            return False
+        if not (x.requires_grad or any(p.requires_grad for p in list(conv.parameters()) + list(tconv.parameters()))):
+            return False
+        B, _, T = x.shape
+        mid, out = tconv.in_channels, tconv.out_channels
+        return bool(H.lib().bm_conv_h2_covers(out, mid, T, 1, 1)) and \
+            bool(H.lib().bm_conv_h2_inop_covers(B, out, mid, T, 1, 1, H.INPUT_OP_ACT))
 
     def forward(self, inputs, batch):
         subjects = batch.subject_index
@@ -186,7 +199,13 @@
                 x = BF.Conv1dFn.apply(x, self.final.weight, self.final.bias, 1, H.ACT_NONE, 0., True)
             else:
                 conv, act, tconv = self.final[0], self.final[1], self.final[2]
-                x = BF.Conv1dFn.apply(x, conv.weight, conv.bias, 1, act.code, act.leak, False)
-                x = BF.Conv1dFn.apply(x, tconv.weight, tconv.bias, 1, H.ACT_NONE, 0., True)
+                if self._head_owns_activation(x, conv, tconv):
+                    x = BF.Conv1dFn.apply(x, conv.weight, conv.bias, 1, H.ACT_NONE, 0., False, 1, None, H.ACT_NONE, 0.,
+                                          False, True)
+                    x = BF.Conv1dFn.apply(x, tconv.weight, tconv.bias, 1, H.ACT_NONE, 0., True, 1, None, act.code,
+                                          act.leak)
+                else:
+                    x = BF.Conv1dFn.apply(x, conv.weight, conv.bias, 1, act.code, act.leak, False)
+                    x = BF.Conv1dFn.apply(x, tconv.weight, tconv.bias, 1, H.ACT_NONE, 0., True)
         assert x.shape[-1] >= length
         return x if x.shape[-1] == length else x[:, :, :length]
diff --git a/include/bm_hip.h b/include/bm_hip.h
--- a/include/bm_hip.h
+++ b/include/bm_hip.h
@@ -84,6 +84,12 @@
                     long res_bstride, float* y_pre, float* y_out, long y_bstride, float* stats, int B, int Cin,
                     int M, int T, int KS, int dil, int act, float leak, int G, float* y_amax_out, float* amax_ws,
                     void* stream);
+int bm_conv_h2_inop_covers(int B, int Cin, int M, int T, int KS, int dil, int kind);
+int bm_conv1d_nn_h2_inop(const float* x, long x_bstride, const float* x_amax, const void* wpacked, const float* bias,
+                         const float* res, long res_bstride, const float* aux, long aux_bstride, float* y,
+                         long y_bstride, float* pairs, int B, int Cin, int M, int T, int KS, int dil, int kind, int act,
+                         float leak, float* y_amax_out, float* amax_ws, float* amax_rows_out, float* sums_out,
+                         void* stream);
 
 int bm_gemm_nt_h2_covers(int M, int Cn, int KS, int S, int T, int G, int dil, int ordered);
 int bm_gemm_nt_h2_suggest_splits(int M, int Cn, int KS, int S, int T);
```

Result: no change. 17260 segments/s (median of 2 runs) (-0.2%).
